# nikkolasg/ark-blst

Measured on AMD Instinct MI355X. Metric: G1 MSM points/sec, higher is better.
Workload: dtype u32; 1 GPU; G1 MSM, 2^20 random bases+scalars per GPU, bases resident, scalars in HBM; points_per_gpu=1048576, total_points=1048576, window_bits=16, num_windows=16, parallelism=base-set sharded x1, scalar_dist=uniform, precomputed_tables=False, bases_validated=True, field_repr=14 x 28-bit limbs in u32 (v_mad_u64_u32)

## Files before the change

ark-blst_amd/binding.py:

```python
from __future__ import annotations

import ctypes as C
import os
import sys

_HERE = os.path.dirname(os.path.abspath(__file__))
SCALAR_CANONICAL, SCALAR_MONTGOMERY = 0, 1
FR_MUL, FR_ADD, FR_SUB = 0, 1, 2
G1_AFF, G1_JAC, G2_AFF, G2_JAC = 96, 144, 192, 288
FP12 = 576
MAX_WINDOWS = 37


ABORT_FN = C.CFUNCTYPE(C.c_int, C.c_void_p)


class WindowInfo(C.Structure):
    _fields_ = [("window_bits", C.c_uint32), ("num_windows", C.c_uint32)]


class MsmError(RuntimeError):
    def __init__(self, code: int, where: str, detail: str = ""):
        self.code = code
        super().__init__(f"{where}: error {code} ({detail})")


class Profile(C.Structure):
    _fields_ = [(n, C.c_double) for n in ("h2d_ms", "ingest_ms", "digits_ms", "scan_ms", "scatter_ms", "accumulate_ms",
                                          "reduce_ms", "combine_ms", "d2h_ms", "host_fold_ms", "total_ms")] + [
        ("window_bits", C.c_uint32), ("num_windows", C.c_uint32), ("n", C.c_uint64), ("accumulate_adds", C.c_uint64),
        ("work_items", C.c_uint32), ("max_items_per_bucket", C.c_uint32),
        ("window_groups", C.c_uint32), ("reserved", C.c_uint32),
        ("accumulate_clock_ghz", C.c_double), ("accumulate_clock_ticks", C.c_uint64), ("accumulate_ref_ticks", C.c_uint64)]


def profile_dict(p: Profile) -> dict:
    return {f: getattr(p, f) for f, _ in Profile._fields_}


class PairingProfile(C.Structure):
    _fields_ = [(n, C.c_double) for n in ("h2d_ms", "lines_ms", "accumulate_ms", "miller_ms", "tree_ms", "host_ms", "total_ms")] + [
        ("n", C.c_uint64), ("pairs_per_accumulator", C.c_uint32), ("reserved", C.c_uint32)]


def lib_path(test_hooks: bool = False) -> str:
    return os.path.join(_HERE, "lib", "libarkblst_amd_test.so" if test_hooks else "libarkblst_amd.so")


_LIBS = {}


def load_library(test_hooks: bool = False):
    if test_hooks not in _LIBS:
        path = lib_path(test_hooks)
        if not os.path.exists(path):
            raise ImportError(f"{path} is missing: run `python -c 'import __graft_entry__ as g; g.build()'` "
                              "(hipcc --offload-arch=gfx950). There is no CPU fallback.")
        L = C.CDLL(path)
        vp, sz, u, i = C.c_void_p, C.c_size_t, C.c_uint, C.c_int
        L.mi_msm_init.argtypes = [C.POINTER(vp), C.POINTER(i), i]
        L.mi_msm_destroy.argtypes = [vp]
        L.mi_msm_destroy.restype = None
        L.mi_msm_num_devices.argtypes = [vp]
        for g in ("g1", "g2"):
            getattr(L, f"mi_msm_{g}_set_bases").argtypes = [vp, vp, sz]
            getattr(L, f"mi_msm_{g}_set_bases_precomputed").argtypes = [vp, vp, sz, u]
            getattr(L, f"mi_msm_{g}_set_bases_device").argtypes = [vp, vp, sz]
            getattr(L, f"mi_msm_{g}_set_bases_from_jacobian").argtypes = [vp, vp, sz]
            getattr(L, f"mi_msm_{g}_set_bases_from_compressed").argtypes = [vp, vp, sz, i, i, C.POINTER(sz)]
            getattr(L, f"mi_{g}_normalize_batch_device").argtypes = [vp, vp, sz, vp]
            getattr(L, f"mi_{g}_deserialize_batch_device").argtypes = [vp, vp, sz, i, i, vp, vp]
            getattr(L, f"mi_{g}_check_batch_device").argtypes = [vp, vp, sz, vp]
            getattr(L, f"mi_msm_{g}_validate_bases").argtypes = [vp, C.POINTER(sz)]
            getattr(L, f"mi_msm_{g}").argtypes = [vp, vp, vp, sz, u, vp]
            getattr(L, f"mi_msm_{g}_device").argtypes = [vp, vp, sz, u, vp]
            getattr(L, f"mi_{g}_sum").argtypes = [vp, sz, vp]
            if hasattr(L, f"mi_msm_{g}_device_windows"):
                getattr(L, f"mi_msm_{g}_device_windows").argtypes = [vp, vp, sz, u, vp, C.POINTER(WindowInfo)]
                getattr(L, f"mi_{g}_fold_windows").argtypes = [vp, sz, sz, C.POINTER(WindowInfo), vp]
            getattr(L, f"mi_msm_{g}_batch").argtypes = [vp, C.POINTER(C.c_char_p), sz, sz, u, vp]
            getattr(L, f"mi_msm_{g}_batch_device").argtypes = [vp, C.POINTER(vp), sz, sz, u, vp]
            getattr(L, f"mi_{g}_normalize_batch").argtypes = [vp, vp, sz, vp]
            if hasattr(L, f"mi_{g}_batch_mul"):
                getattr(L, f"mi_{g}_batch_mul").argtypes = [vp, vp, vp, sz, u, vp]
                getattr(L, f"mi_{g}_batch_mul_device").argtypes = [vp, vp, vp, sz, u, vp]
        if hasattr(L, "mi_batch_mul_set_window_bits"):
            L.mi_batch_mul_set_window_bits.argtypes = [vp, u]
        if hasattr(L, "mi_fr_ntt"):
            L.mi_fr_ntt.argtypes = [vp, vp, u, sz, i, vp, u, vp]
            L.mi_fr_ntt_device.argtypes = [vp, vp, u, sz, i, vp, u, vp]
            L.mi_fr_vec_op_device.argtypes = [vp, i, vp, vp, sz, u, vp]
        for g in ("g1", "g2"):
            getattr(L, f"mi_{g}_deserialize_batch").argtypes = [vp, vp, sz, i, i, vp, vp]
            getattr(L, f"mi_{g}_serialize_batch").argtypes = [vp, vp, sz, i, vp]
            getattr(L, f"mi_{g}_check_batch").argtypes = [vp, vp, sz, vp]
        L.mi_multi_miller_loop.argtypes = [vp, vp, vp, sz, vp]
        L.mi_multi_pairing.argtypes = [vp, vp, vp, sz, vp]
        L.mi_final_exponentiation.argtypes = [vp, vp]
        L.mi_msm_set_window_bits.argtypes = [vp, u]
        L.mi_msm_get_window_bits.argtypes = [vp, C.POINTER(u)]
        L.mi_msm_set_abort_check.argtypes = [vp, ABORT_FN, vp]
        L.mi_msm_set_pipeline.argtypes = [vp, C.POINTER(u), u]
        L.mi_msm_set_base_cache.argtypes = [vp, u]
        L.mi_msm_invalidate_base_cache.argtypes = [vp]
        L.mi_msm_base_cache_stats.argtypes = [vp, C.POINTER(C.c_uint64), C.POINTER(C.c_uint64), C.POINTER(u)]
        L.mi_msm_device_id.argtypes = [vp, i]
        L.mi_msm_set_profile_level.argtypes = [vp, i]
        L.mi_msm_last_profile.argtypes = [vp, C.POINTER(Profile)]
        if hasattr(L, "mi_pairing_last_profile"):
            L.mi_pairing_last_profile.argtypes = [vp, C.POINTER(PairingProfile)]
        L.mi_msm_last_error.argtypes = [vp]
        L.mi_msm_last_error.restype = C.c_char_p
        L.mi_msm_strerror.argtypes = [i]
        L.mi_msm_strerror.restype = C.c_char_p
        if test_hooks:
            L.mi_test_fp_op.argtypes = [vp, i, vp, vp, vp, sz]
            L.mi_test_field_op.argtypes = [vp, i, vp, sz, vp]
            L.mi_test_field_op_info.argtypes = [i, C.POINTER(i), C.POINTER(i), C.POINTER(i)]
            L.mi_test_field_op_info.restype = C.c_char_p
            L.mi_test_set_pairing.argtypes = [vp, u, u, i]
            L.mi_test_set_max_part.argtypes = [vp, sz]
            L.mi_test_fail_allocs.argtypes = [i]
            L.mi_test_fail_allocs.restype = None
            L.mi_test_set_no_peer.argtypes = [vp, i]
            L.mi_test_plan.argtypes = [sz, u, i, i, sz, C.POINTER(C.c_uint32)]
        _LIBS[test_hooks] = L
    return _LIBS[test_hooks]


def _buf(b):
    if b is None:
        return None, None
    if isinstance(b, int):
        return C.c_void_p(b), None
    if isinstance(b, bytes):
        return C.cast(C.c_char_p(b), C.c_void_p), b
    mv = memoryview(b)
    arr = (C.c_char * mv.nbytes).from_buffer(mv) if not mv.readonly else (C.c_char * mv.nbytes).from_buffer_copy(mv)
    return C.cast(arr, C.c_void_p), arr


def check_runtime_order():
    torch = sys.modules.get("torch")
    if torch is None or os.environ.get("ARKBLST_AMD_SKIP_RUNTIME_ORDER_CHECK"):
        return
    tlib = os.path.join(os.path.dirname(getattr(torch, "__file__", "") or ""), "lib")
    if not os.path.exists(os.path.join(tlib, "libamdhip64.so")) and not any(f.startswith("libamdhip64.so") for f in (os.listdir(tlib) if os.path.isdir(tlib) else [])):
        return
    try:
        mapped = {line.split()[-1] for line in open("/proc/self/maps") if "libamdhip64.so" in line}
    except OSError:
        return
    foreign = sorted(m for m in mapped if not os.path.realpath(m).startswith(os.path.realpath(tlib)))
    if foreign:
        raise ImportError("libarkblst_amd.so was loaded before torch: the process holds TWO HIP runtimes (" + ", ".join(sorted(mapped)) + "); torch's bundled "
                          "one under " + tlib + " then finds no devices ('No HIP GPUs are available').  Import torch BEFORE the first ark_blst_amd "
                          "context is created (INTEGRATION.md §6); ARKBLST_AMD_SKIP_RUNTIME_ORDER_CHECK=1 silences this check.")


class Context:

    def __init__(self, device_ids=None, test_hooks: bool = False):
        self._L = load_library(test_hooks)
        check_runtime_order()
        self._h = C.c_void_p()
        if device_ids is None:
            device_ids = [0]
        ids = (C.c_int * len(device_ids))(*device_ids)
        rc = self._L.mi_msm_init(C.byref(self._h), ids, len(device_ids))
        if rc != 0:
            raise MsmError(rc, "mi_msm_init", self._L.mi_msm_strerror(rc).decode())

    def close(self):
        if self._h:
            self._L.mi_msm_destroy(self._h)
            self._h = C.c_void_p()

    def __del__(self):
        try:
            self.close()
        except Exception:
            pass

    def __enter__(self):
        return self

    def __exit__(self, *a):
        self.close()

    def _check(self, rc, where):
        if rc != 0:
            raise MsmError(rc, where, (self._L.mi_msm_last_error(self._h) or b"").decode())

    def num_devices(self) -> int:
        return self._L.mi_msm_num_devices(self._h)

    def set_window_bits(self, c: int):
        self._check(self._L.mi_msm_set_window_bits(self._h, c), "mi_msm_set_window_bits")

    def set_abort_check(self, fn=None):
        self._abort_cb = ABORT_FN(lambda _user: 1 if fn() else 0) if fn else C.cast(None, ABORT_FN)
        self._check(self._L.mi_msm_set_abort_check(self._h, self._abort_cb, None), "mi_msm_set_abort_check")

    def get_window_bits(self) -> int:
        v = C.c_uint(0)
        self._check(self._L.mi_msm_get_window_bits(self._h, C.byref(v)), "mi_msm_get_window_bits")
        return v.value

    def set_pipeline(self, weights=None):
        w = list(weights or [])
        arr = (C.c_uint * max(1, len(w)))(*w)
        self._check(self._L.mi_msm_set_pipeline(self._h, arr, len(w)), "mi_msm_set_pipeline")

    def set_base_cache(self, entries: int):
        self._check(self._L.mi_msm_set_base_cache(self._h, entries), "mi_msm_set_base_cache")

    def invalidate_base_cache(self):
        self._check(self._L.mi_msm_invalidate_base_cache(self._h), "mi_msm_invalidate_base_cache")

    def base_cache_stats(self) -> dict:
        h, m, e = C.c_uint64(0), C.c_uint64(0), C.c_uint(0)
        self._check(self._L.mi_msm_base_cache_stats(self._h, C.byref(h), C.byref(m), C.byref(e)), "mi_msm_base_cache_stats")
        return {"hits": h.value, "misses": m.value, "entries": e.value}

    def device_id(self, slot: int = 0) -> int:
        return self._L.mi_msm_device_id(self._h, slot)

    def set_profile_level(self, level: int):
        self._check(self._L.mi_msm_set_profile_level(self._h, level), "mi_msm_set_profile_level")

    def set_bases(self, group: str, bases, n: int):
        p, keep = _buf(bases)
        self._check(getattr(self._L, f"mi_msm_{group}_set_bases")(self._h, p, n), f"mi_msm_{group}_set_bases")

    def set_bases_precomputed(self, group: str, bases, n: int, window_bits: int = 0):
        p, keep = _buf(bases)
        self._check(getattr(self._L, f"mi_msm_{group}_set_bases_precomputed")(self._h, p, n, window_bits),
                    f"mi_msm_{group}_set_bases_precomputed")

    def set_bases_device(self, group: str, d_bases_ptr: int, n: int):
        self._check(getattr(self._L, f"mi_msm_{group}_set_bases_device")(self._h, C.c_void_p(d_bases_ptr), n), f"mi_msm_{group}_set_bases_device")

    def set_bases_from_jacobian(self, group: str, jac, n: int):
        p, keep = _buf(jac)
        self._check(getattr(self._L, f"mi_msm_{group}_set_bases_from_jacobian")(self._h, p, n), f"mi_msm_{group}_set_bases_from_jacobian")

    def set_bases_from_compressed(self, group: str, data, n: int, compressed: bool = True, validate: bool = True) -> int:
        p, keep = _buf(data)
        rej = C.c_size_t(0)
        rc = getattr(self._L, f"mi_msm_{group}_set_bases_from_compressed")(self._h, p, n, 1 if compressed else 0, 1 if validate else 0, C.byref(rej))
        if rc != 0 and not (rc == -1 and rej.value):
            self._check(rc, f"mi_msm_{group}_set_bases_from_compressed")
        return rej.value

    def normalize_batch_device(self, group: str, d_in_ptr: int, n: int, d_out_ptr: int):
        self._check(getattr(self._L, f"mi_{group}_normalize_batch_device")(self._h, C.c_void_p(d_in_ptr), n, C.c_void_p(d_out_ptr)), f"mi_{group}_normalize_batch_device")

    def deserialize_batch_device(self, group: str, d_bytes_ptr: int, n: int, compressed: bool, validate: bool, d_out_ptr: int, d_status_ptr: int):
        self._check(getattr(self._L, f"mi_{group}_deserialize_batch_device")(self._h, C.c_void_p(d_bytes_ptr), n, 1 if compressed else 0,
                                                                              1 if validate else 0, C.c_void_p(d_out_ptr), C.c_void_p(d_status_ptr)),
                    f"mi_{group}_deserialize_batch_device")

    def check_batch_device(self, group: str, d_points_ptr: int, n: int, d_status_ptr: int):
        self._check(getattr(self._L, f"mi_{group}_check_batch_device")(self._h, C.c_void_p(d_points_ptr), n, C.c_void_p(d_status_ptr)), f"mi_{group}_check_batch_device")

    def validate_bases(self, group: str) -> int:
        bad = C.c_size_t(0)
        self._check(getattr(self._L, f"mi_msm_{group}_validate_bases")(self._h, C.byref(bad)), "mi_msm_validate_bases")
        return bad.value

    def msm(self, group: str, bases, scalars, n: int, scalar_fmt: int = SCALAR_CANONICAL) -> bytes:
        out = C.create_string_buffer(G1_JAC if group == "g1" else G2_JAC)
        pb, kb = _buf(bases)
        ps, ks = _buf(scalars)
        self._check(getattr(self._L, f"mi_msm_{group}")(self._h, pb, ps, n, scalar_fmt, out), f"mi_msm_{group}")
        return out.raw

    def msm_batch(self, group: str, scalar_vectors, n: int, scalar_fmt: int = SCALAR_CANONICAL):
        k = len(scalar_vectors)
        size = G1_JAC if group == "g1" else G2_JAC
        out = C.create_string_buffer(size * max(k, 1))
        arr = (C.c_char_p * max(k, 1))(*[bytes(v) for v in scalar_vectors])
        self._check(getattr(self._L, f"mi_msm_{group}_batch")(self._h, arr, k, n, scalar_fmt, out), f"mi_msm_{group}_batch")
        return [out.raw[size * j:size * (j + 1)] for j in range(k)]

    def msm_batch_device(self, group: str, d_scalar_ptrs, n: int, scalar_fmt: int = SCALAR_CANONICAL):
        k = len(d_scalar_ptrs)
        size = G1_JAC if group == "g1" else G2_JAC
        out = C.create_string_buffer(size * max(k, 1))
        arr = (C.c_void_p * max(k, 1))(*[C.c_void_p(p) for p in d_scalar_ptrs])
        self._check(getattr(self._L, f"mi_msm_{group}_batch_device")(self._h, arr, k, n, scalar_fmt, out), f"mi_msm_{group}_batch_device")
        return [out.raw[size * j:size * (j + 1)] for j in range(k)]

    def msm_device(self, group: str, d_scalars_ptr: int, n: int, scalar_fmt: int = SCALAR_CANONICAL) -> bytes:
        out = C.create_string_buffer(G1_JAC if group == "g1" else G2_JAC)
        self._check(getattr(self._L, f"mi_msm_{group}_device")(self._h, C.c_void_p(d_scalars_ptr), n, scalar_fmt, out),
                    f"mi_msm_{group}_device")
        return out.raw

    def msm_device_windows(self, group: str, d_scalars_ptr: int, n: int, scalar_fmt: int, d_out_ptr: int):
        info = WindowInfo()
        self._check(getattr(self._L, f"mi_msm_{group}_device_windows")(self._h, C.c_void_p(d_scalars_ptr), n, scalar_fmt,
                                                                        C.c_void_p(d_out_ptr), C.byref(info)), f"mi_msm_{group}_device_windows")
        return int(info.window_bits), int(info.num_windows)

    def normalize_batch(self, group: str, jac: bytes, into=None):
        jb, ab = (G1_JAC, G1_AFF) if group == "g1" else (G2_JAC, G2_AFF)
        n = len(jac) // jb
        if into is not None:
            po, ko = _buf(into)
            self._check(getattr(self._L, f"mi_{group}_normalize_batch")(self._h, jac, n, po), f"mi_{group}_normalize_batch")
            return into
        out = C.create_string_buffer(ab * n)
        self._check(getattr(self._L, f"mi_{group}_normalize_batch")(self._h, jac, n, out), f"mi_{group}_normalize_batch")
        return out.raw

    def batch_mul(self, group: str, base, scalars, scalar_fmt: int = SCALAR_CANONICAL, into=None):
        ab = G1_AFF if group == "g1" else G2_AFF
        n = len(scalars) // 32
        pb, kb = _buf(base)
        ps, ks = _buf(scalars)
        if into is not None:
            po, ko = _buf(into)
            self._check(getattr(self._L, f"mi_{group}_batch_mul")(self._h, pb, ps, n, scalar_fmt, po), f"mi_{group}_batch_mul")
            return into
        out = C.create_string_buffer(ab * max(n, 1))
        self._check(getattr(self._L, f"mi_{group}_batch_mul")(self._h, pb, ps, n, scalar_fmt, out), f"mi_{group}_batch_mul")
        return out.raw[:ab * n]

    def batch_mul_device(self, group: str, base, d_scalars_ptr: int, n: int, scalar_fmt: int, d_out_ptr: int):
        pb, kb = _buf(base)
        self._check(getattr(self._L, f"mi_{group}_batch_mul_device")(self._h, pb, C.c_void_p(d_scalars_ptr), n, scalar_fmt, C.c_void_p(d_out_ptr)),
                    f"mi_{group}_batch_mul_device")

    def set_batch_mul_window_bits(self, w: int):
        self._check(self._L.mi_batch_mul_set_window_bits(self._h, w), "mi_batch_mul_set_window_bits")

    def fr_ntt(self, data, log_n: int, batch: int = 1, inverse: bool = False, coset_offset=None, scalar_fmt: int = SCALAR_MONTGOMERY, into=None):
        nbytes = (batch << log_n) * 32 if 0 <= log_n <= 26 and batch > 0 else 0
        pd, kd = _buf(data)
        pc, kc = _buf(coset_offset)
        if into is not None:
            po, ko = _buf(into)
            self._check(self._L.mi_fr_ntt(self._h, pd, log_n, batch, int(inverse), pc, scalar_fmt, po), "mi_fr_ntt")
            return into
        out = C.create_string_buffer(max(nbytes, 1))
        self._check(self._L.mi_fr_ntt(self._h, pd, log_n, batch, int(inverse), pc, scalar_fmt, out), "mi_fr_ntt")
        return out.raw[:nbytes]

    def fr_ntt_device(self, d_in_ptr: int, log_n: int, batch: int, inverse: bool, coset_offset, scalar_fmt: int, d_out_ptr: int):
        pc, kc = _buf(coset_offset)
        self._check(self._L.mi_fr_ntt_device(self._h, C.c_void_p(d_in_ptr), log_n, batch, int(inverse), pc, scalar_fmt, C.c_void_p(d_out_ptr)), "mi_fr_ntt_device")

    def fr_vec_op_device(self, op: int, d_a_ptr: int, d_b_ptr: int, n: int, scalar_fmt: int, d_out_ptr: int):
        self._check(self._L.mi_fr_vec_op_device(self._h, op, C.c_void_p(d_a_ptr), C.c_void_p(d_b_ptr), n, scalar_fmt, C.c_void_p(d_out_ptr)), "mi_fr_vec_op_device")

    def deserialize_batch(self, group: str, data: bytes, compressed: bool = True, validate: bool = True, into=None):
        unit = 48 if group == "g1" else 96
        size = unit if compressed else 2 * unit
        n = len(data) // size
        if into is not None:
            po, ko = _buf(into[0])
            ps, ks = _buf(into[1])
            self._check(getattr(self._L, f"mi_{group}_deserialize_batch")(self._h, data, n, int(compressed), int(validate), po, ps),
                        f"mi_{group}_deserialize_batch")
            return into
        out = C.create_string_buffer(2 * unit * n)
        st = C.create_string_buffer(n)
        self._check(getattr(self._L, f"mi_{group}_deserialize_batch")(self._h, data, n, int(compressed), int(validate), out, st),
                    f"mi_{group}_deserialize_batch")
        return out.raw, st.raw

    def check_batch(self, group: str, points: bytes) -> bytes:
        aff = G1_AFF if group == "g1" else G2_AFF
        n = len(points) // aff
        st = C.create_string_buffer(n)
        p, keep = _buf(points)
        self._check(getattr(self._L, f"mi_{group}_check_batch")(self._h, p, n, st), f"mi_{group}_check_batch")
        return st.raw

    def serialize_batch(self, group: str, points: bytes, compressed: bool = True) -> bytes:
        unit = 48 if group == "g1" else 96
        n = len(points) // (2 * unit)
        out = C.create_string_buffer((unit if compressed else 2 * unit) * n)
        self._check(getattr(self._L, f"mi_{group}_serialize_batch")(self._h, points, n, int(compressed), out), f"mi_{group}_serialize_batch")
        return out.raw

    def g1_deserialize_batch(self, data: bytes, compressed: bool = True, validate: bool = True):
        return self.deserialize_batch("g1", data, compressed, validate)

    def g1_serialize_batch(self, points: bytes, compressed: bool = True) -> bytes:
        return self.serialize_batch("g1", points, compressed)

    def multi_miller_loop(self, g1_affine: bytes, g2_affine: bytes) -> bytes:
        n = len(g1_affine) // G1_AFF
        assert len(g1_affine) == n * G1_AFF and len(g2_affine) == n * G2_AFF, "one G2 point per G1 point"
        out = C.create_string_buffer(FP12)
        self._check(self._L.mi_multi_miller_loop(self._h, g1_affine, g2_affine, n, out), "mi_multi_miller_loop")
        return out.raw

    def multi_pairing(self, g1_affine: bytes, g2_affine: bytes) -> bytes:
        n = len(g1_affine) // G1_AFF
        assert len(g1_affine) == n * G1_AFF and len(g2_affine) == n * G2_AFF, "one G2 point per G1 point"
        out = C.create_string_buffer(FP12)
        self._check(self._L.mi_multi_pairing(self._h, g1_affine, g2_affine, n, out), "mi_multi_pairing")
        return out.raw

    def profile(self) -> dict:
        return profile_dict(self.profile_raw())

    def profile_raw(self) -> Profile:
        p = Profile()
        self._check(self._L.mi_msm_last_profile(self._h, C.byref(p)), "mi_msm_last_profile")
        return p

    def pairing_profile(self) -> dict:
        p = PairingProfile()
        self._check(self._L.mi_pairing_last_profile(self._h, C.byref(p)), "mi_pairing_last_profile")
        return {f: getattr(p, f) for f, _ in PairingProfile._fields_ if f != "reserved"}

    def test_fp_op(self, op: int, a: bytes, b: bytes) -> bytes:
        n = len(a) // 48
        out = C.create_string_buffer(48 * n)
        self._check(self._L.mi_test_fp_op(self._h, op, a, b, out, n), "mi_test_fp_op")
        return out.raw

    def test_field_op(self, op: int, data: bytes, n: int) -> bytes:
        in_slots, out_slots = C.c_int(0), C.c_int(0)
        if not self._L.mi_test_field_op_info(op, C.byref(in_slots), C.byref(out_slots), None):
            raise ValueError(f"no field op {op}")
        if len(data) != 64 * in_slots.value * n:
            raise ValueError(f"field op {op}: {n} elements take {64 * in_slots.value * n} bytes of operands, got {len(data)}")
        out = C.create_string_buffer(64 * out_slots.value * n)
        self._check(self._L.mi_test_field_op(self._h, op, data, n, out), "mi_test_field_op")
        return out.raw

    def test_field_ops(self):
        ops, a, b, k = [], C.c_int(0), C.c_int(0), C.c_int(0)
        while True:
            name = self._L.mi_test_field_op_info(len(ops), C.byref(a), C.byref(b), C.byref(k))
            if not name:
                return ops
            ops.append((name.decode(), a.value, b.value, k.value))

    def test_set_pairing(self, share: int = 0, batch: int = 0, single_lane: bool = False):
        self._check(self._L.mi_test_set_pairing(self._h, share, batch, int(single_lane)), "mi_test_set_pairing")

    def test_set_max_part(self, points: int):
        self._check(self._L.mi_test_set_max_part(self._h, points), "mi_test_set_max_part")

    def test_fail_allocs(self, count: int):
        self._L.mi_test_fail_allocs(count)

    def test_set_no_peer(self, no_peer: bool):
        self._check(self._L.mi_test_set_no_peer(self._h, int(no_peer)), "mi_test_set_no_peer")


def test_plan(n: int, forced_c: int = 0, group: str = "g1", shared: bool = False, stride: int = 0, fold: bool = False) -> dict:
    out = (C.c_uint32 * 13)()
    rc = load_library(True).mi_test_plan(n, forced_c, 0 if group == "g1" else 1, int(shared) | (2 if fold else 0), stride, out)
    if rc != 0:
        raise MsmError(rc, "mi_test_plan")
    keys = ("c", "nwin", "bwin", "coop_L", "chunk_buckets", "logT", "lo_bits", "serial", "chunks_per_win")
    d = {k: int(out[i]) for i, k in enumerate(keys)}
    d["nbuckets"] = (int(out[9]) << 32) | int(out[10])
    d["nchunks"] = int(out[11])
    d["serial_L"] = int(out[12])
    d["serial_reduce"] = d["serial"]
    return d


def final_exponentiation(f: bytes) -> bytes:
    assert len(f) == FP12
    out = C.create_string_buffer(FP12)
    rc = load_library().mi_final_exponentiation(f, out)
    if rc != 0:
        raise MsmError(rc, "mi_final_exponentiation")
    return out.raw


def _sum(group: str, partials) -> bytes:
    L = load_library()
    size = G1_JAC if group == "g1" else G2_JAC
    blob = b"".join(partials)
    assert len(blob) % size == 0
    out = C.create_string_buffer(size)
    rc = getattr(L, f"mi_{group}_sum")(blob, len(blob) // size, out)
    if rc != 0:
        raise MsmError(rc, f"mi_{group}_sum")
    return out.raw


def fold_windows(group: str, windows, n_ranks: int, rank_stride: int, window_bits: int, num_windows: int) -> bytes:
    size = G1_JAC if group == "g1" else G2_JAC
    p, keep = _buf(windows)
    assert memoryview(windows).nbytes >= n_ranks * rank_stride * size or n_ranks * num_windows == 0
    info = WindowInfo(window_bits, num_windows)
    out = C.create_string_buffer(size)
    rc = getattr(load_library(), f"mi_{group}_fold_windows")(p, n_ranks, rank_stride, C.byref(info), out)
    if rc != 0:
        raise MsmError(rc, f"mi_{group}_fold_windows")
    return out.raw


def g1_sum(partials) -> bytes:
    return _sum("g1", partials)


def g2_sum(partials) -> bytes:
    return _sum("g2", partials)


class RcclTiming(C.Structure):
    _fields_ = [("msm_ms", C.c_double), ("exchange_ms", C.c_double), ("window_bits", C.c_uint32), ("num_windows", C.c_uint32),
                ("repeats", C.c_uint32), ("bytes_per_rank", C.c_uint32)]


RCCL_UNIQUE_ID_BYTES = 128
_RCCL = []


def rccl_lib_path() -> str:
    return os.path.join(_HERE, "lib", "libarkblst_amd_rccl.so")


def load_rccl_library():
    if not _RCCL:
        load_library(False)
        path = rccl_lib_path()
        if not os.path.exists(path):
            raise ImportError(f"{path} is missing: run `python -c 'import __graft_entry__ as g; g.build()'`")
        L = C.CDLL(path)
        vp, sz, u, i = C.c_void_p, C.c_size_t, C.c_uint, C.c_int
        L.mi_rccl_get_unique_id.argtypes = [vp]
        L.mi_rccl_comm_create.argtypes = [C.POINTER(vp), vp, vp, i, i]
        L.mi_rccl_comm_attach.argtypes = [C.POINTER(vp), vp, vp]
        L.mi_rccl_comm_set_timeout_ms.argtypes = [vp, C.c_double]
        L.mi_rccl_comm_destroy.argtypes = [vp]
        L.mi_rccl_comm_destroy.restype = None
        L.mi_rccl_comm_size.argtypes = [vp]
        L.mi_rccl_comm_rank.argtypes = [vp]
        for g in ("g1", "g2"):
            getattr(L, f"mi_msm_{g}_allgather_fold").argtypes = [vp, vp, sz, u, vp]
        L.mi_rccl_last_timing.argtypes = [vp, C.POINTER(RcclTiming)]
        L.mi_rccl_last_error.restype = C.c_char_p
        _RCCL.append(L)
    return _RCCL[0]


def rccl_unique_id() -> bytes:
    L = load_rccl_library()
    buf = C.create_string_buffer(RCCL_UNIQUE_ID_BYTES)
    rc = L.mi_rccl_get_unique_id(buf)
    if rc != 0:
        raise MsmError(rc, "mi_rccl_get_unique_id", (L.mi_rccl_last_error() or b"").decode())
    return buf.raw


class RcclComm:

    def __init__(self, ctx: Context, unique_id: bytes, n_ranks: int, rank: int):
        self._L = load_rccl_library()
        self._h = C.c_void_p()
        self._ctx = ctx
        rc = self._L.mi_rccl_comm_create(C.byref(self._h), ctx._h, unique_id, n_ranks, rank)
        if rc != 0:
            raise MsmError(rc, "mi_rccl_comm_create", (self._L.mi_rccl_last_error() or b"").decode())

    def close(self):
        if self._h:
            self._L.mi_rccl_comm_destroy(self._h)
            self._h = C.c_void_p()

    def __enter__(self):
        return self

    def __exit__(self, *a):
        self.close()

    def set_timeout_ms(self, ms: float):
        rc = self._L.mi_rccl_comm_set_timeout_ms(self._h, float(ms))
        if rc != 0:
            raise MsmError(rc, "mi_rccl_comm_set_timeout_ms", (self._L.mi_rccl_last_error() or b"").decode())

    def size(self) -> int:
        return self._L.mi_rccl_comm_size(self._h)

    def rank(self) -> int:
        return self._L.mi_rccl_comm_rank(self._h)

    def allgather_fold(self, group: str, d_scalars_ptr: int, n: int, scalar_fmt: int = SCALAR_CANONICAL) -> bytes:
        out = C.create_string_buffer(G1_JAC if group == "g1" else G2_JAC)
        rc = getattr(self._L, f"mi_msm_{group}_allgather_fold")(self._h, C.c_void_p(d_scalars_ptr), n, scalar_fmt, out)
        if rc != 0:
            raise MsmError(rc, f"mi_msm_{group}_allgather_fold", (self._L.mi_rccl_last_error() or b"").decode())
        return out.raw

    def timing_raw(self) -> RcclTiming:
        t = RcclTiming()
        self._L.mi_rccl_last_timing(self._h, C.byref(t))
        return t

    def timing(self) -> dict:
        t = self.timing_raw()
        return {f: getattr(t, f) for f, _ in RcclTiming._fields_}
```

ark-blst_amd/csrc/api.hip:

```cpp
#include <random>
#include "internal.hpp"
#if defined(MI_TEST_HOOKS)
#include "test_hooks.h"
namespace mi { std::atomic<int> g_fail_allocs{0}; }
#endif

using namespace mi;

namespace {
bool cpu_ok() {
#if defined(__x86_64__)
    static const bool ok = __builtin_cpu_supports("bmi2") && __builtin_cpu_supports("adx");
    return ok;
#else
    return true;
#endif
}

template <class J, class Raw>
int fold_windows(const Raw* windows, size_t n_ranks, size_t rank_stride, const mi_window_info* info, Raw* out) {
    if (!out || !info || (n_ranks && info->num_windows && !windows)) return MI_E_INVALID;
    if (info->num_windows > MI_MAX_WINDOWS || rank_stride < info->num_windows ||
        (info->num_windows && (info->window_bits < 1 || info->window_bits > 32)))
        return MI_E_INVALID;
    if (!cpu_ok()) return MI_E_UNSUPPORTED;
    static_assert(sizeof(J) == sizeof(Raw), "host Jacobian type must be the reference's layout");
    J r = J::inf();
    for (int w = (int)info->num_windows - 1; w >= 0; w--) {
        r = r.dbl_n(info->window_bits);
        for (size_t k = 0; k < n_ranks; k++) {
            J p;
            memcpy(&p, &windows[k * rank_stride + (size_t)w], sizeof p);
            r = r.add(p);
        }
    }
    memcpy(out, &r, sizeof r);
    return MI_OK;
}
}

extern "C" {

int mi_msm_init(mi_ctx** out, const int* device_ids, int n_devices) {
    if (!out || n_devices < 0) return MI_E_INVALID;
    *out = nullptr;
    if (!cpu_ok()) return MI_E_UNSUPPORTED;
    int count = 0;
    if (hipGetDeviceCount(&count) != hipSuccess || count <= 0) return MI_E_NO_DEVICE;
    if (n_devices == 0) n_devices = device_ids ? 0 : count;
    if (n_devices <= 0 || (!device_ids && n_devices > count) || n_devices > 64) return MI_E_NO_DEVICE;
    mi_ctx* ctx = new (std::nothrow) mi_ctx();
    if (!ctx) return MI_E_NOMEM;
    int rc = guarded(ctx, [&]() -> int {
        ctx->devs.resize(n_devices);
        ctx->devs_b.resize(n_devices);
        ctx->residents.resize(n_devices);
        for (int k = 0; k < n_devices; k++) {
            int id = device_ids ? device_ids[k] : k;
            if (id < 0 || id >= count) return MI_E_NO_DEVICE;
            HIP_TRY(hipSetDevice(id));
            for (DevState* d : {&ctx->devs[k], &ctx->devs_b[k]}) {
                d->dev = id;
                d->res = ctx->residents[k].data();
                int cus = 0;
                if (hipDeviceGetAttribute(&cus, hipDeviceAttributeMultiprocessorCount, id) == hipSuccess && cus > 0) d->simds = 4u * (uint32_t)cus;
                HIP_TRY(hipStreamCreateWithFlags(&d->stream, hipStreamNonBlocking));
                HIP_TRY(hipStreamCreateWithFlags(&d->copy_stream, hipStreamNonBlocking));
                for (auto& e : d->ev) HIP_TRY(hipEventCreate(&e));
                for (auto& e : d->cev) HIP_TRY(hipEventCreate(&e));
                for (Scratch& sc : d->sc)
                    for (auto& e : sc.ev) HIP_TRY(hipEventCreate(&e));
                for (auto& row : d->iev)
                    for (auto& e : row) HIP_TRY(hipEventCreate(&e));
            }
        }
        if (const char* e = getenv("ARKBLST_AMD_TRACE")) ctx->trace = atoi(e) != 0;
        if (const char* e = getenv("ARKBLST_AMD_PIPELINE_ACC2")) ctx->pipe_two_acc_streams = atoi(e) != 0;
        if (const char* e = getenv("ARKBLST_AMD_PIPELINE")) {
            std::vector<unsigned> w;
            if (!strcmp(e, "0") || !strcmp(e, "off") || !strcmp(e, "1")) w = {1};
            else if (strcmp(e, "auto"))
                for (const char* q = e; *q;) {
                    char* end = nullptr;
                    unsigned long v = strtoul(q, &end, 10);
                    if (end == q) break;
                    w.push_back((unsigned)std::min<unsigned long>(std::max<unsigned long>(v, 1), 1000));
                    q = *end == ',' ? end + 1 : end;
                    if (*end && *end != ',') break;
                }
            if (w.size() > (size_t)MAX_GROUPS) w.resize(MAX_GROUPS);
            ctx->pipe_weights = w;
        }
        {
            std::random_device rd;
            ctx->hash_seed = ((uint64_t)rd() << 32) | rd();
            ctx->hash_mult = (((uint64_t)rd() << 32) | rd()) | 0x8000000000000001ull;
        }
        if (const char* e = getenv("ARKBLST_AMD_BASE_CACHE")) {
            long v = strtol(e, nullptr, 10);
            ctx->cache_entries = (unsigned)std::min<long>(std::max<long>(v, 0), MI_BASE_CACHE_MAX);
            ctx->cache_env = true;
        }
        if (n_devices > 1) {
            for (int l = 0; l < NLANES; l++) ctx->workers[l].reset(new DeviceWorkers((size_t)n_devices));
            for (int a = 0; a < n_devices; a++)
                for (int b = 0; b < n_devices; b++) {
                    int da = ctx->devs[a].dev, db = ctx->devs[b].dev, can = 0;
                    if (da == db) continue;
                    if (hipDeviceCanAccessPeer(&can, da, db) == hipSuccess && can) {
                        (void)hipSetDevice(da);
                        if (hipDeviceEnablePeerAccess(db, 0) != hipSuccess) (void)hipGetLastError();
                    } else {
                        (void)hipGetLastError();
                    }
                }
        }
        return MI_OK;
    });
    if (rc != MI_OK) {
        mi_msm_destroy(ctx);
        return rc;
    }
    *out = ctx;
    return MI_OK;
}

void mi_msm_destroy(mi_ctx* ctx) {
    if (!ctx) return;
    ctx->batch_workers.reset();
    for (int l = 0; l < NLANES; l++) ctx->workers[l].reset();
    for (std::vector<DevState>* lane : {&ctx->devs, &ctx->devs_b})
        for (auto& d : *lane) {
            (void)hipSetDevice(d.dev);
            if (d.stream) (void)hipStreamSynchronize(d.stream);
            if (d.acc2_stream) (void)hipStreamSynchronize(d.acc2_stream);
            if (d.aux_stream) (void)hipStreamSynchronize(d.aux_stream);
            d.for_each_buf([](DevBuf& b) { b.release(); });
            if (d.h_pairs) (void)hipHostFree(d.h_pairs);
            for (auto& e : d.ev)
                if (e) (void)hipEventDestroy(e);
            for (auto& e : d.cev)
                if (e) (void)hipEventDestroy(e);
            for (Scratch& sc : d.sc) {
                if (sc.h_meta) (void)hipHostFree(sc.h_meta);
                for (auto& e : sc.ev)
                    if (e) (void)hipEventDestroy(e);
            }
            for (auto& row : d.iev)
                for (auto& e : row)
                    if (e) (void)hipEventDestroy(e);
            if (d.d2h_stream) { (void)hipStreamSynchronize(d.d2h_stream); (void)hipStreamDestroy(d.d2h_stream); }
            if (d.aux_stream) (void)hipStreamDestroy(d.aux_stream);
            if (d.acc2_stream) (void)hipStreamDestroy(d.acc2_stream);
            if (d.copy_stream) (void)hipStreamDestroy(d.copy_stream);
            if (d.stream) (void)hipStreamDestroy(d.stream);
        }
    for (auto& v : ctx->cache) v.clear();
    if (!ctx->devs.empty()) {
        (void)hipSetDevice(ctx->devs[0].dev);
        for (FixedTable& t : ctx->fb) t.buf.release();
        for (FrTable& t : ctx->ntt_tables) { t.lo.release(); t.hi.release(); }
        ctx->ntt_scratch.release();
    }
    for (size_t k = 0; k < ctx->residents.size() && k < ctx->devs.size(); k++) {
        (void)hipSetDevice(ctx->devs[k].dev);
        for (Resident& x : ctx->residents[k]) { x.buf.release(); x.flags.release(); }
    }
    delete ctx;
}

int mi_msm_num_devices(const mi_ctx* ctx) { return ctx ? (int)ctx->devs.size() : 0; }
int mi_msm_device_id(const mi_ctx* ctx, int slot) { return ctx && slot >= 0 && (size_t)slot < ctx->devs.size() ? ctx->devs[(size_t)slot].dev : -1; }

int mi_msm_g1_set_bases(mi_ctx* ctx, const mi_g1_affine* bases, size_t n) { return g1_set_bases(ctx, bases, n, 0); }
int mi_msm_g2_set_bases(mi_ctx* ctx, const mi_g2_affine* bases, size_t n) { return g2_set_bases(ctx, bases, n, 0); }
int mi_msm_g1_set_bases_precomputed(mi_ctx* ctx, const mi_g1_affine* bases, size_t n, unsigned window_bits) {
    return g1_set_bases(ctx, bases, n, window_bits ? window_bits : 1);
}
int mi_msm_g2_set_bases_precomputed(mi_ctx* ctx, const mi_g2_affine* bases, size_t n, unsigned window_bits) {
    return g2_set_bases(ctx, bases, n, window_bits ? window_bits : 1);
}

int mi_msm_g1_validate_bases(mi_ctx* ctx, size_t* n_invalid) { return g1_validate_bases(ctx, n_invalid); }
int mi_msm_g2_validate_bases(mi_ctx* ctx, size_t* n_invalid) { return g2_validate_bases(ctx, n_invalid); }

int mi_msm_g1(mi_ctx* ctx, const mi_g1_affine* bases, const uint8_t* scalars, size_t n, unsigned scalar_fmt, mi_g1* out) {
    return g1_msm(ctx, bases, scalars, false, n, scalar_fmt, out);
}
int mi_msm_g2(mi_ctx* ctx, const mi_g2_affine* bases, const uint8_t* scalars, size_t n, unsigned scalar_fmt, mi_g2* out) {
    return g2_msm(ctx, bases, scalars, false, n, scalar_fmt, out);
}
int mi_msm_g1_device(mi_ctx* ctx, const void* d_scalars, size_t n, unsigned scalar_fmt, mi_g1* out) {
    return g1_msm(ctx, nullptr, static_cast<const uint8_t*>(d_scalars), true, n, scalar_fmt, out);
}
int mi_msm_g2_device(mi_ctx* ctx, const void* d_scalars, size_t n, unsigned scalar_fmt, mi_g2* out) {
    return g2_msm(ctx, nullptr, static_cast<const uint8_t*>(d_scalars), true, n, scalar_fmt, out);
}

int mi_msm_g1_device_windows(mi_ctx* ctx, const void* d_scalars, size_t n, unsigned scalar_fmt, void* d_out_windows, mi_window_info* info) {
    return g1_msm_windows(ctx, static_cast<const uint8_t*>(d_scalars), n, scalar_fmt, d_out_windows, info);
}
int mi_msm_g2_device_windows(mi_ctx* ctx, const void* d_scalars, size_t n, unsigned scalar_fmt, void* d_out_windows, mi_window_info* info) {
    return g2_msm_windows(ctx, static_cast<const uint8_t*>(d_scalars), n, scalar_fmt, d_out_windows, info);
}
int mi_g1_fold_windows(const mi_g1* windows, size_t n_ranks, size_t rank_stride, const mi_window_info* info, mi_g1* out) {
    return fold_windows<hostec::G1>(windows, n_ranks, rank_stride, info, out);
}
int mi_g2_fold_windows(const mi_g2* windows, size_t n_ranks, size_t rank_stride, const mi_window_info* info, mi_g2* out) {
    return fold_windows<hostec::G2>(windows, n_ranks, rank_stride, info, out);
}

int mi_msm_g1_batch(mi_ctx* ctx, const uint8_t* const* scalars, size_t k, size_t n, unsigned scalar_fmt, mi_g1* out) {
    return g1_msm_batch(ctx, scalars, false, k, n, scalar_fmt, out);
}
int mi_msm_g2_batch(mi_ctx* ctx, const uint8_t* const* scalars, size_t k, size_t n, unsigned scalar_fmt, mi_g2* out) {
    return g2_msm_batch(ctx, scalars, false, k, n, scalar_fmt, out);
}
int mi_msm_g1_batch_device(mi_ctx* ctx, const void* const* d_scalars, size_t k, size_t n, unsigned scalar_fmt, mi_g1* out) {
    return g1_msm_batch(ctx, reinterpret_cast<const uint8_t* const*>(d_scalars), true, k, n, scalar_fmt, out);
}
int mi_msm_g2_batch_device(mi_ctx* ctx, const void* const* d_scalars, size_t k, size_t n, unsigned scalar_fmt, mi_g2* out) {
    return g2_msm_batch(ctx, reinterpret_cast<const uint8_t* const*>(d_scalars), true, k, n, scalar_fmt, out);
}

int mi_g1_normalize_batch(mi_ctx* ctx, const mi_g1* in, size_t n, mi_g1_affine* out) { return g1_normalize(ctx, in, false, n, out); }
int mi_g2_normalize_batch(mi_ctx* ctx, const mi_g2* in, size_t n, mi_g2_affine* out) { return g2_normalize(ctx, in, false, n, out); }
int mi_g1_normalize_batch_device(mi_ctx* ctx, const void* d_in, size_t n, void* d_out) {
    return g1_normalize(ctx, static_cast<const mi_g1*>(d_in), true, n, static_cast<mi_g1_affine*>(d_out));
}
int mi_g2_normalize_batch_device(mi_ctx* ctx, const void* d_in, size_t n, void* d_out) {
    return g2_normalize(ctx, static_cast<const mi_g2*>(d_in), true, n, static_cast<mi_g2_affine*>(d_out));
}
int mi_msm_g1_set_bases_device(mi_ctx* ctx, const void* d_bases, size_t n) { return g1_set_bases_device(ctx, d_bases, n); }
int mi_msm_g2_set_bases_device(mi_ctx* ctx, const void* d_bases, size_t n) { return g2_set_bases_device(ctx, d_bases, n); }
int mi_msm_g1_set_bases_from_jacobian(mi_ctx* ctx, const mi_g1* points, size_t n) { return g1_set_bases_from_jacobian(ctx, points, n); }
int mi_msm_g2_set_bases_from_jacobian(mi_ctx* ctx, const mi_g2* points, size_t n) { return g2_set_bases_from_jacobian(ctx, points, n); }
int mi_msm_g1_set_bases_from_compressed(mi_ctx* ctx, const uint8_t* bytes, size_t n, int compressed, int validate, size_t* n_rejected) {
    return g1_set_bases_from_compressed(ctx, bytes, n, compressed, validate, n_rejected);
}
int mi_msm_g2_set_bases_from_compressed(mi_ctx* ctx, const uint8_t* bytes, size_t n, int compressed, int validate, size_t* n_rejected) {
    return g2_set_bases_from_compressed(ctx, bytes, n, compressed, validate, n_rejected);
}

int mi_g1_deserialize_batch(mi_ctx* ctx, const uint8_t* bytes, size_t n, int compressed, int validate, mi_g1_affine* out,
                            uint8_t* status) {
    return g1_deserialize(ctx, bytes, false, n, compressed, validate, out, status);
}
int mi_g1_deserialize_batch_device(mi_ctx* ctx, const void* d_bytes, size_t n, int compressed, int validate, void* d_out, void* d_status) {
    return g1_deserialize(ctx, static_cast<const uint8_t*>(d_bytes), true, n, compressed, validate, static_cast<mi_g1_affine*>(d_out), static_cast<uint8_t*>(d_status));
}
int mi_g2_deserialize_batch_device(mi_ctx* ctx, const void* d_bytes, size_t n, int compressed, int validate, void* d_out, void* d_status) {
    return g2_deserialize(ctx, static_cast<const uint8_t*>(d_bytes), true, n, compressed, validate, static_cast<mi_g2_affine*>(d_out), static_cast<uint8_t*>(d_status));
}
int mi_g1_serialize_batch(mi_ctx* ctx, const mi_g1_affine* points, size_t n, int compressed, uint8_t* bytes) {
    return g1_serialize(ctx, points, n, compressed, bytes);
}
int mi_g2_deserialize_batch(mi_ctx* ctx, const uint8_t* bytes, size_t n, int compressed, int validate, mi_g2_affine* out,
                            uint8_t* status) {
    return g2_deserialize(ctx, bytes, false, n, compressed, validate, out, status);
}
int mi_g2_serialize_batch(mi_ctx* ctx, const mi_g2_affine* points, size_t n, int compressed, uint8_t* bytes) {
    return g2_serialize(ctx, points, n, compressed, bytes);
}

int mi_g1_check_batch(mi_ctx* ctx, const mi_g1_affine* points, size_t n, uint8_t* status) { return g1_check_batch(ctx, points, false, n, status); }
int mi_g2_check_batch(mi_ctx* ctx, const mi_g2_affine* points, size_t n, uint8_t* status) { return g2_check_batch(ctx, points, false, n, status); }
int mi_g1_check_batch_device(mi_ctx* ctx, const void* d_points, size_t n, void* d_status) {
    return g1_check_batch(ctx, static_cast<const mi_g1_affine*>(d_points), true, n, static_cast<uint8_t*>(d_status));
}
int mi_g2_check_batch_device(mi_ctx* ctx, const void* d_points, size_t n, void* d_status) {
    return g2_check_batch(ctx, static_cast<const mi_g2_affine*>(d_points), true, n, static_cast<uint8_t*>(d_status));
}

int mi_g1_batch_mul(mi_ctx* ctx, const mi_g1_affine* base, const uint8_t* scalars, size_t n, unsigned scalar_fmt, mi_g1_affine* out) {
    return g1_batch_mul(ctx, base, scalars, false, n, scalar_fmt, out);
}
int mi_g2_batch_mul(mi_ctx* ctx, const mi_g2_affine* base, const uint8_t* scalars, size_t n, unsigned scalar_fmt, mi_g2_affine* out) {
    return g2_batch_mul(ctx, base, scalars, false, n, scalar_fmt, out);
}
int mi_g1_batch_mul_device(mi_ctx* ctx, const mi_g1_affine* base, const void* d_scalars, size_t n, unsigned scalar_fmt, void* d_out) {
    return g1_batch_mul(ctx, base, static_cast<const uint8_t*>(d_scalars), true, n, scalar_fmt, static_cast<mi_g1_affine*>(d_out));
}
int mi_g2_batch_mul_device(mi_ctx* ctx, const mi_g2_affine* base, const void* d_scalars, size_t n, unsigned scalar_fmt, void* d_out) {
    return g2_batch_mul(ctx, base, static_cast<const uint8_t*>(d_scalars), true, n, scalar_fmt, static_cast<mi_g2_affine*>(d_out));
}
int mi_batch_mul_set_window_bits(mi_ctx* ctx, unsigned window_bits) { return batch_mul_set_window_bits(ctx, window_bits); }

int mi_fr_ntt(mi_ctx* ctx, const uint8_t* in, unsigned log_n, size_t batch, int inverse, const uint8_t* coset_offset, unsigned scalar_fmt, uint8_t* out) {
    return fr_ntt(ctx, in, false, log_n, batch, inverse, coset_offset, scalar_fmt, out);
}
int mi_fr_ntt_device(mi_ctx* ctx, const void* d_in, unsigned log_n, size_t batch, int inverse, const uint8_t* coset_offset, unsigned scalar_fmt, void* d_out) {
    return fr_ntt(ctx, static_cast<const uint8_t*>(d_in), true, log_n, batch, inverse, coset_offset, scalar_fmt, static_cast<uint8_t*>(d_out));
}
int mi_fr_vec_op_device(mi_ctx* ctx, int op, const void* d_a, const void* d_b, size_t n, unsigned scalar_fmt, void* d_out) {
    return fr_vec_op(ctx, op, d_a, d_b, n, scalar_fmt, d_out);
}

int mi_multi_miller_loop(mi_ctx* ctx, const mi_g1_affine* p, const mi_g2_affine* q, size_t n, mi_fp12* out) {
    return miller(ctx, p, q, n, out, false);
}
int mi_multi_pairing(mi_ctx* ctx, const mi_g1_affine* p, const mi_g2_affine* q, size_t n, mi_fp12* out) {
    return miller(ctx, p, q, n, out, true);
}
int mi_final_exponentiation(const mi_fp12* f, mi_fp12* out) { return cpu_ok() ? final_exponentiation(f, out) : MI_E_UNSUPPORTED; }

int mi_g1_sum(const mi_g1* partials, size_t n, mi_g1* out) {
    if (!out || (n && !partials)) return MI_E_INVALID;
    if (!cpu_ok()) return MI_E_UNSUPPORTED;
    hostec::G1 r = hostec::G1::inf();
    for (size_t i = 0; i < n; i++) {
        hostec::G1 p;
        memcpy(&p, &partials[i], sizeof p);
        r = r.add(p);
    }
    memcpy(out, &r, sizeof r);
    return MI_OK;
}

int mi_g2_sum(const mi_g2* partials, size_t n, mi_g2* out) {
    if (!out || (n && !partials)) return MI_E_INVALID;
    if (!cpu_ok()) return MI_E_UNSUPPORTED;
    hostec::G2 r = hostec::G2::inf();
    for (size_t i = 0; i < n; i++) {
        hostec::G2 p;
        memcpy(&p, &partials[i], sizeof p);
        r = r.add(p);
    }
    memcpy(out, &r, sizeof r);
    return MI_OK;
}

int mi_msm_set_base_cache(mi_ctx* ctx, unsigned entries) {
    if (!ctx || entries > MI_BASE_CACHE_MAX) return fail(ctx, MI_E_INVALID, "entries must be 0..MI_BASE_CACHE_MAX");
    DeviceRestore restore;
    std::vector<std::shared_ptr<BaseCacheEntry>> dropped;
    {
        std::lock_guard<std::mutex> lk(ctx->cache_mu);
        if (ctx->cache_env) return MI_OK;
        ctx->cache_entries = entries;
        for (auto& v : ctx->cache)
            while (v.size() > entries) { dropped.push_back(v.back()); v.pop_back(); }
    }
    return MI_OK;
}

int mi_msm_invalidate_base_cache(mi_ctx* ctx) {
    if (!ctx) return MI_E_INVALID;
    DeviceRestore restore;
    std::vector<std::shared_ptr<BaseCacheEntry>> dropped;
    {
        std::lock_guard<std::mutex> lk(ctx->cache_mu);
        for (auto& v : ctx->cache) { for (auto& e : v) dropped.push_back(e); v.clear(); }
    }
    return MI_OK;
}

int mi_msm_base_cache_stats(const mi_ctx* ctx, uint64_t* hits, uint64_t* misses, unsigned* entries_in_use) {
    if (!ctx) return MI_E_INVALID;
    mi_ctx* c = const_cast<mi_ctx*>(ctx);
    std::lock_guard<std::mutex> lk(c->cache_mu);
    if (hits) *hits = c->cache_hits;
    if (misses) *misses = c->cache_misses;
    if (entries_in_use) *entries_in_use = (unsigned)(c->cache[0].size() + c->cache[1].size());
    return MI_OK;
}

int mi_msm_set_window_bits(mi_ctx* ctx, unsigned window_bits) {
    if (!ctx || (window_bits != 0 && (window_bits < 7 || window_bits > 22))) return fail(ctx, MI_E_INVALID, "window_bits must be 0 or 7..22");
    LaneLock lk(ctx, true);
    ctx->forced_c = window_bits;
    return MI_OK;
}

int mi_msm_set_abort_check(mi_ctx* ctx, int (*check)(void*), void* user) {
    if (!ctx) return MI_E_INVALID;
    LaneLock lk(ctx, true);
    ctx->abort_check = check;
    ctx->abort_user = user;
    return MI_OK;
}

int mi_msm_get_window_bits(const mi_ctx* ctx, unsigned* window_bits) {
    if (!ctx || !window_bits) return MI_E_INVALID;
    LaneLock lk(const_cast<mi_ctx*>(ctx), true);
    *window_bits = ctx->forced_c;
    return MI_OK;
}

int mi_msm_set_pipeline(mi_ctx* ctx, const unsigned* weights, unsigned n_groups) {
    if (!ctx || n_groups > (unsigned)MAX_GROUPS || (n_groups > 1 && !weights)) return fail(ctx, MI_E_INVALID, "at most 4 window groups; weights must be given for more than one");
    LaneLock lk(ctx, true);
    ctx->pipe_weights.clear();
    if (n_groups == 1) ctx->pipe_weights = {1};
    for (unsigned g = 0; n_groups > 1 && g < n_groups; g++) ctx->pipe_weights.push_back(std::min(std::max(weights[g], 1u), 1000u));
    return MI_OK;
}

int mi_msm_set_profile_level(mi_ctx* ctx, int level) {
    if (!ctx || level < 0 || level > 2) return fail(ctx, MI_E_INVALID, "profile level must be 0, 1 or 2");
    LaneLock lk(ctx, true);
    ctx->profile_level = level;
    return MI_OK;
}

int mi_msm_last_profile(const mi_ctx* ctx, mi_profile* out) {
    if (!ctx || !out) return MI_E_INVALID;
    std::lock_guard<std::mutex> lk(ctx->info_mu);
    *out = ctx->prof;
    return MI_OK;
}

int mi_pairing_last_profile(const mi_ctx* ctx, mi_pairing_profile* out) {
    if (!ctx || !out) return MI_E_INVALID;
    std::lock_guard<std::mutex> lk(ctx->info_mu);
    *out = ctx->pprof;
    return MI_OK;
}

const char* mi_msm_last_error(const mi_ctx* ctx) {
    (void)ctx;
    return tls_error().c_str();
}

const char* mi_msm_strerror(int code) {
    switch (code) {
        case MI_OK: return "ok";
        case MI_E_INVALID: return "invalid argument";
        case MI_E_NO_DEVICE: return "no usable HIP device";
        case MI_E_HIP: return "HIP runtime error";
        case MI_E_NOMEM: return "out of memory";
        case MI_E_NO_BASES: return "no resident base set";
        case MI_E_UNSUPPORTED: return "not supported on this host (the library needs an x86-64 CPU with BMI2 and ADX)";
        case MI_E_COMM: return "RCCL communication error";
        case MI_E_ABORTED: return "aborted by the caller's abort check";
        default: return "unknown error";
    }
}

#if defined(MI_TEST_HOOKS)
int mi_test_fp_op(mi_ctx* ctx, int op, const mi_fp* a, const mi_fp* b, mi_fp* out, size_t n) { return test_fp_op(ctx, op, a, b, out, n); }
int mi_test_field_op(mi_ctx* ctx, int op, const uint32_t* in, size_t n, uint32_t* out) { return test_field_op(ctx, op, in, n, out); }
const char* mi_test_field_op_info(int op, int* in_slots, int* out_slots, int* kind) { return test_field_op_info(op, in_slots, out_slots, kind); }
int mi_test_set_pairing(mi_ctx* ctx, unsigned share, unsigned batch, int single_lane) {
    if (!ctx) return MI_E_INVALID;
    LaneLock lk(ctx, true);
    ctx->test_pairing_share = share;
    ctx->test_pairing_batch = batch;
    ctx->test_pairing_single_lane = single_lane != 0;
    return MI_OK;
}
int mi_test_set_max_part(mi_ctx* ctx, size_t points) {
    if (!ctx) return MI_E_INVALID;
    LaneLock lk(ctx, true);
    ctx->test_max_part = points;
    return MI_OK;
}
void mi_test_fail_allocs(int count) { g_fail_allocs.store(count); }
int mi_test_set_no_peer(mi_ctx* ctx, int no_peer) {
    if (!ctx) return MI_E_INVALID;
    LaneLock lk(ctx, true);
    ctx->test_no_peer = no_peer != 0;
    return MI_OK;
}
int mi_test_plan(size_t n, unsigned forced_c, int group, int shared, size_t stride, uint32_t* out) {
    if (!out || n == 0) return MI_E_INVALID;
    Plan p = make_plan(n, forced_c, group == 0 ? g1_cost() : g2_cost(), (shared & 1) != 0, stride, (shared & 2) != 0);
    out[0] = p.c; out[1] = p.nwin; out[2] = p.bwin; out[3] = p.coop_L; out[4] = p.chunk_buckets; out[5] = p.logT; out[6] = p.lo_bits;
    out[7] = p.serial_reduce ? 1u : 0u; out[8] = p.chunks_per_win; out[9] = (uint32_t)(p.nbuckets >> 32); out[10] = (uint32_t)p.nbuckets;
    out[11] = (uint32_t)p.nchunks; out[12] = p.serial_reduce ? p.serial_L : 0u;
    return MI_OK;
}
#endif

}
```

ark-blst_amd/csrc/common.hpp:

```cpp
#pragma once
#include <hip/hip_runtime.h>

#include <algorithm>
#include <array>
#include <atomic>
#include <chrono>
#include <condition_variable>
#include <cstdarg>
#include <cstdio>
#include <cstdlib>
#include <cstring>
#include <functional>
#include <memory>
#include <mutex>
#include <new>
#include <string>
#include <thread>
#include <vector>

#include "../../include/arkblst_amd.h"
#include "host_curve.hpp"

namespace mi {

struct HipFail {
    std::string msg;
    bool oom = false;
    bool invalid = false;
    bool aborted = false;
};
#define HIP_TRY(expr)                                                                                     \
    do {                                                                                                  \
        hipError_t _e = (expr);                                                                           \
        if (_e != hipSuccess) {                                                                           \
            char _b[512];                                                                                 \
            snprintf(_b, sizeof _b, "%s failed: %s (%s:%d)", #expr, hipGetErrorString(_e), __FILE__, __LINE__); \
            throw ::mi::HipFail{_b, _e == hipErrorOutOfMemory};                                           \
        }                                                                                                 \
    } while (0)

#if defined(MI_TEST_HOOKS)
extern std::atomic<int> g_fail_allocs;
#endif

inline uint32_t num_windows(unsigned c, bool fold) { return (255 + c - 1) / c + ((!fold && 255 % c == 0) ? 1u : 0u); }

struct Plan {
    uint32_t c, nwin;
    uint32_t win0;
    bool fold;
    uint32_t bwin;
    uint32_t nb, coop_L, chunks_per_win, logT, lo_bits;
    uint32_t logS;
    uint32_t cls_shift;
    uint64_t nbuckets, nchunks;
    uint32_t chunk_buckets;
    bool serial_reduce;
    uint32_t serial_L;
};

struct DevBuf {
    void* p = nullptr;
    size_t cap = 0;
    void ensure(size_t bytes) {
        if (bytes <= cap) return;
#if defined(MI_TEST_HOOKS)
        if (g_fail_allocs.load() > 0 && g_fail_allocs.fetch_sub(1) > 0) throw HipFail{"injected allocation failure (test hook): out of memory", true};
#endif
        if (p) HIP_TRY(hipFree(p));
        p = nullptr;
        cap = 0;
        HIP_TRY(hipMalloc(&p, bytes));
        cap = bytes;
    }
    void release() {
        if (p) (void)hipFree(p);
        p = nullptr;
        cap = 0;
    }
    void ensure_fit(size_t bytes) {
        if (cap > 2 * bytes && cap - bytes > ((size_t)64 << 20)) release();
        ensure(bytes);
    }
};

struct Resident {
    DevBuf buf, flags;
    size_t n = 0;
    size_t lo = 0;
    uint32_t tables = 1;
    uint32_t table_c = 0;
    bool validated = false;
};

struct FixedTable {
    DevBuf buf;
    std::vector<uint8_t> key;
    unsigned w = 0;
    bool valid = false;
    uint64_t builds = 0;
};

struct FrTable {
    bool coset = false;
    unsigned log_n = 0;
    int inverse = 0;
    uint8_t key[32] = {};
    DevBuf lo, hi;
    unsigned h = 0;
    uint64_t stamp = 0;
};
constexpr size_t FR_TABLES_KEPT = 8;

struct Fp128 {
    uint64_t a = 0, b = 0;
    bool operator==(const Fp128& o) const { return a == o.a && b == o.b; }
    bool operator!=(const Fp128& o) const { return !(*this == o); }
};

struct BaseCacheEntry {
    const void* ptr = nullptr;
    size_t n = 0;
    Fp128 fp;
    uint64_t stamp = 0;
    std::vector<Resident> shard;
    std::vector<int> devs;
    ~BaseCacheEntry() {
        for (size_t k = 0; k < shard.size(); k++) {
            if (!shard[k].buf.p && !shard[k].flags.p) continue;
            (void)hipSetDevice(devs[k]);
            shard[k].buf.release();
            shard[k].flags.release();
        }
    }
};

constexpr int MAX_GROUPS = 4;
struct Scratch {
    DevBuf hist, offsets, woff, meta, sched, sorted, partial, order, item_bucket, pairs, pairs2;
    DevBuf tilecnt, tileoff, bin_tot, bin_base, binA_base, coarse, coarseA, seg_cnt, seg_base, segcnt, segoff, merge_list, merge_list2;
    uint32_t* h_meta = nullptr;
    hipEvent_t ev[8] = {};
    template <class Fn> void for_each_buf(Fn fn) {
        for (DevBuf* b : {&hist, &offsets, &woff, &meta, &sched, &sorted, &partial, &order, &item_bucket, &pairs, &pairs2, &tilecnt, &tileoff, &bin_tot,
                          &bin_base, &binA_base, &coarse, &coarseA, &seg_cnt, &seg_base, &segcnt, &segoff, &merge_list, &merge_list2})
            fn(*b);
    }
};

struct DevState {
    int dev = 0;
    uint32_t simds = 1024;
    hipStream_t stream = nullptr;
    hipStream_t copy_stream = nullptr;
    hipStream_t acc2_stream = nullptr, aux_stream = nullptr;
    hipStream_t d2h_stream = nullptr;
    hipEvent_t ev[12] = {};
    hipEvent_t cev[10] = {};
    hipEvent_t iev[4][8] = {};
    Resident* res = nullptr;
    DevBuf raw, call_bases, call_flags, scalars;
    Scratch sc[MAX_GROUPS];
    DevBuf pr_p, pr_q, pr_lvl[2], pr_raw, pr_lines;
    DevBuf io_in, io_out, io_status, nv_vals, nv_pref, nv_inv, nv_top;
    DevBuf fb_jac;
    void* h_pairs = nullptr;
    size_t h_pairs_cap = 0;
    mi_profile prof{};
    int prof_level = 1;

    void ensure_host(size_t bytes) {
        if (bytes <= h_pairs_cap) return;
        if (h_pairs) (void)hipHostFree(h_pairs);
        h_pairs = nullptr;
        h_pairs_cap = 0;
        HIP_TRY(hipHostMalloc(&h_pairs, bytes, hipHostMallocDefault));
        h_pairs_cap = bytes;
    }
    static int high_priority() {
        int lo = 0, hi = 0;
        HIP_TRY(hipDeviceGetStreamPriorityRange(&lo, &hi));
        return hi;
    }
    void ensure_pipeline_streams() {
        if (aux_stream) return;
        HIP_TRY(hipStreamCreateWithFlags(&acc2_stream, hipStreamNonBlocking));
        HIP_TRY(hipStreamCreateWithPriority(&aux_stream, hipStreamNonBlocking, high_priority()));
    }
    void ensure_d2h_stream() {
        if (!d2h_stream) HIP_TRY(hipStreamCreateWithPriority(&d2h_stream, hipStreamNonBlocking, high_priority()));
    }
    template <class Fn> void for_each_buf(Fn fn) {
        for (DevBuf* b : {&raw, &call_bases, &call_flags, &scalars, &pr_p, &pr_q, &pr_lvl[0], &pr_lvl[1], &pr_raw, &pr_lines, &io_in, &io_out, &io_status,
                          &nv_vals, &nv_pref, &nv_inv, &nv_top, &fb_jac})
            fn(*b);
        for (Scratch& s : sc) s.for_each_buf(fn);
    }
};

constexpr int NLANES = 2;
class HashPool;

class DeviceWorkers {
public:
    explicit DeviceWorkers(size_t n) : slots_(n) {
        for (size_t k = 0; k < n; k++) threads_.emplace_back([this, k] { loop(k); });
    }
    ~DeviceWorkers() {
        {
            std::lock_guard<std::mutex> lk(mu_);
            stop_ = true;
        }
        cv_.notify_all();
        for (auto& t : threads_) t.join();
    }
    DeviceWorkers(const DeviceWorkers&) = delete;
    DeviceWorkers& operator=(const DeviceWorkers&) = delete;
    size_t size() const { return threads_.size(); }
    void run(const std::function<void(size_t)>& fn) {
        std::unique_lock<std::mutex> lk(mu_);
        fn_ = &fn;
        pending_ = slots_.size();
        for (auto& s : slots_) s = true;
        cv_.notify_all();
        done_cv_.wait(lk, [&] { return pending_ == 0; });
        fn_ = nullptr;
    }

private:
    void loop(size_t k) {
        for (;;) {
            const std::function<void(size_t)>* fn;
            {
                std::unique_lock<std::mutex> lk(mu_);
                cv_.wait(lk, [&] { return stop_ || slots_[k]; });
                if (stop_) return;
                slots_[k] = false;
                fn = fn_;
            }
            (*fn)(k);
            {
                std::lock_guard<std::mutex> lk(mu_);
                if (--pending_ == 0) done_cv_.notify_all();
            }
        }
    }
    std::vector<std::thread> threads_;
    std::vector<char> slots_;
    std::mutex mu_;
    std::condition_variable cv_, done_cv_;
    const std::function<void(size_t)>* fn_ = nullptr;
    size_t pending_ = 0;
    bool stop_ = false;
};

}

struct mi_ctx {
    std::vector<mi::DevState> devs;
    std::vector<mi::DevState> devs_b;
    std::vector<std::array<mi::Resident, 2>> residents;
    std::unique_ptr<mi::DeviceWorkers> workers[mi::NLANES];
    std::unique_ptr<mi::DeviceWorkers> batch_workers;
    std::mutex batch_mu;
    std::mutex lane_mu;
    std::condition_variable lane_cv;
    bool lane_busy[mi::NLANES] = {false, false};
    mutable std::mutex info_mu;
    unsigned forced_c = 0;
    unsigned fb_forced_w = 0;
    mi::FixedTable fb[2];
    std::vector<mi::FrTable> ntt_tables;
    uint64_t ntt_clock = 0;
    mi::DevBuf ntt_scratch;
    std::vector<unsigned> pipe_weights;
    int (*abort_check)(void*) = nullptr;
    void* abort_user = nullptr;
    bool pipe_two_acc_streams = false;
    bool trace = false;
    std::mutex cache_mu;
    unsigned cache_entries = 0;
    bool cache_env = false;
    uint64_t cache_clock = 0, cache_hits = 0, cache_misses = 0;
    std::vector<std::shared_ptr<mi::BaseCacheEntry>> cache[2];
    uint64_t hash_seed = 0, hash_mult = 0xD6E8FEB86659FD93ull;
    std::shared_ptr<mi::HashPool> hash_pool[mi::NLANES];
    int profile_level = 1;
    mi_profile prof{};
    mi_pairing_profile pprof{};
    std::string err;
#if defined(MI_TEST_HOOKS)
    unsigned test_pairing_share = 0, test_pairing_batch = 0;
    bool test_pairing_single_lane = false;
    size_t test_max_part = 0;
    bool test_no_peer = false;
#endif
};

namespace mi {

struct HashKey { uint64_t seed = 0, mult = 0xD6E8FEB86659FD93ull; };
struct SliceHash { uint64_t h[4]; };
inline SliceHash hash_slice(const uint8_t* p, size_t bytes, uint64_t slice, const HashKey& key) {
    const uint64_t K = key.mult | 1u, seed = key.seed + slice * 0x9E3779B97F4A7C15ull;
    SliceHash s{{0x9E3779B97F4A7C15ull ^ seed, 0xC2B2AE3D27D4EB4Full + seed, 0x165667B19E3779F9ull ^ (seed << 1), 0x27D4EB2F165667C5ull + (seed << 2)}};
    size_t i = 0;
    for (; i + 32 <= bytes; i += 32) {
        uint64_t w[4];
        memcpy(w, p + i, 32);
        for (int t = 0; t < 4; t++) {
            s.h[t] = (s.h[t] ^ w[t]) * K;
            s.h[t] ^= s.h[t] >> 32;
        }
    }
    if (i < bytes) {
        uint64_t w[4] = {0, 0, 0, 0};
        memcpy(w, p + i, bytes - i);
        for (int t = 0; t < 4; t++) {
            s.h[t] = (s.h[t] ^ w[t] ^ (uint64_t)(bytes - i)) * K;
            s.h[t] ^= s.h[t] >> 32;
        }
    }
    return s;
}
inline Fp128 fold_slices(const SliceHash* s, size_t count, uint64_t total_bytes) {
    Fp128 r{0x243F6A8885A308D3ull ^ total_bytes, 0x13198A2E03707344ull + total_bytes};
    for (size_t k = 0; k < count; k++)
        for (int t = 0; t < 4; t++) {
            r.a = (r.a ^ s[k].h[t]) * 0xD6E8FEB86659FD93ull;
            r.a ^= r.a >> 29;
            r.b = (r.b + s[k].h[t]) * 0x9FB21C651E98DF25ull;
            r.b ^= r.b >> 31;
        }
    return r;
}
constexpr size_t HASH_SLICE_MIN = (size_t)1 << 20;
inline size_t hash_slices(size_t bytes, size_t threads) { return std::max<size_t>(1, std::min(threads, bytes / HASH_SLICE_MIN)); }
inline Fp128 content_fingerprint(const uint8_t* p, size_t bytes, size_t threads, const HashKey& key = HashKey{}) {
    const size_t S = hash_slices(bytes, threads);
    std::vector<SliceHash> part(S);
    for (size_t k = 0; k < S; k++) {
        const size_t lo = (bytes / 32 * k / S) * 32, hi = k + 1 == S ? bytes : (bytes / 32 * (k + 1) / S) * 32;
        part[k] = hash_slice(p + lo, hi - lo, (uint64_t)k, key);
    }
    return fold_slices(part.data(), S, bytes);
}

class HashPool {
public:
    explicit HashPool(size_t threads, const HashKey& key = HashKey{}) : key_(key), part_(std::max<size_t>(1, threads)) {
        for (size_t k = 0; k < part_.size(); k++) threads_.emplace_back([this, k] { loop(k); });
    }
    ~HashPool() {
        {
            std::lock_guard<std::mutex> lk(mu_);
            stop_ = true;
        }
        cv_.notify_all();
        for (auto& t : threads_) t.join();
    }
    HashPool(const HashPool&) = delete;
    HashPool& operator=(const HashPool&) = delete;
    size_t threads() const { return part_.size(); }
    bool busy() const { return busy_; }
    void start(const uint8_t* p, size_t bytes) {
        std::lock_guard<std::mutex> lk(mu_);
        p_ = p; bytes_ = bytes;
        slices_ = hash_slices(bytes, part_.size());
        pending_ = slices_;
        gen_++;
        busy_ = true;
        cv_.notify_all();
    }
    Fp128 finish() {
        std::unique_lock<std::mutex> lk(mu_);
        done_cv_.wait(lk, [&] { return pending_ == 0; });
        busy_ = false;
        return fold_slices(part_.data(), slices_, bytes_);
    }

private:
    void loop(size_t k) {
        uint64_t seen = 0;
        for (;;) {
            const uint8_t* p;
            size_t bytes, S;
            {
                std::unique_lock<std::mutex> lk(mu_);
                cv_.wait(lk, [&] { return stop_ || gen_ != seen; });
                if (stop_) return;
                seen = gen_;
                p = p_; bytes = bytes_; S = slices_;
            }
            if (k >= S) continue;
            const size_t lo = (bytes / 32 * k / S) * 32, hi = k + 1 == S ? bytes : (bytes / 32 * (k + 1) / S) * 32;
            const SliceHash h = hash_slice(p + lo, hi - lo, (uint64_t)k, key_);
            {
                std::lock_guard<std::mutex> lk(mu_);
                part_[k] = h;
                if (--pending_ == 0) done_cv_.notify_all();
            }
        }
    }
    const HashKey key_;
    std::vector<SliceHash> part_;
    std::vector<std::thread> threads_;
    std::mutex mu_;
    std::condition_variable cv_, done_cv_;
    const uint8_t* p_ = nullptr;
    size_t bytes_ = 0, slices_ = 0, pending_ = 0;
    uint64_t gen_ = 0;
    bool stop_ = false, busy_ = false;
};
inline size_t hash_pool_threads() {
    if (const char* e = getenv("ARKBLST_AMD_HASH_THREADS")) return (size_t)std::min(16l, std::max(1l, atol(e)));
    return std::min<size_t>(6, std::max<size_t>(1, std::thread::hardware_concurrency() / 3));
}

inline bool cache_begin(mi_ctx* ctx, int idx, const void* ptr, size_t n, std::shared_ptr<BaseCacheEntry>& candidate) {
    std::lock_guard<std::mutex> lk(ctx->cache_mu);
    if (!ctx->cache_entries) return false;
    for (auto& e : ctx->cache[idx])
        if (e->ptr == ptr && e->n == n && (!candidate || e->stamp > candidate->stamp)) candidate = e;
    return true;
}
inline std::shared_ptr<BaseCacheEntry> cache_find(mi_ctx* ctx, int idx, const void* ptr, size_t n, const Fp128& fp) {
    std::lock_guard<std::mutex> lk(ctx->cache_mu);
    for (auto& e : ctx->cache[idx])
        if (e->ptr == ptr && e->n == n && e->fp == fp) return e;
    return nullptr;
}
inline void cache_finish(mi_ctx* ctx, int idx, const std::shared_ptr<BaseCacheEntry>& hit, const std::shared_ptr<BaseCacheEntry>& fill, const Fp128& fp) {
    std::vector<std::shared_ptr<BaseCacheEntry>> dropped;
    std::lock_guard<std::mutex> lk(ctx->cache_mu);
    auto& v = ctx->cache[idx];
    if (hit) {
        hit->stamp = ++ctx->cache_clock;
        ctx->cache_hits++;
        return;
    }
    ctx->cache_misses++;
    if (!fill) return;
    fill->fp = fp;
    bool dup = false;
    for (auto& e : v) dup = dup || (e->ptr == fill->ptr && e->n == fill->n && e->fp == fill->fp);
    if (dup || !ctx->cache_entries) return;
    fill->stamp = ++ctx->cache_clock;
    v.push_back(fill);
    while (v.size() > ctx->cache_entries) {
        size_t old = 0;
        for (size_t q = 1; q < v.size(); q++)
            if (v[q]->stamp < v[old]->stamp) old = q;
        dropped.push_back(v[old]);
        v.erase(v.begin() + (long)old);
    }
}

struct LaneLock {
    mi_ctx* c;
    int lane;
    LaneLock(mi_ctx* ctx, bool exclusive) : c(ctx), lane(-1) {
        std::unique_lock<std::mutex> lk(c->lane_mu);
        if (exclusive) {
            c->lane_cv.wait(lk, [&] { return !c->lane_busy[0] && !c->lane_busy[1]; });
            c->lane_busy[0] = c->lane_busy[1] = true;
        } else {
            c->lane_cv.wait(lk, [&] { return !c->lane_busy[0] || !c->lane_busy[1]; });
            lane = c->lane_busy[0] ? 1 : 0;
            c->lane_busy[lane] = true;
        }
    }
    ~LaneLock() {
        {
            std::lock_guard<std::mutex> lk(c->lane_mu);
            if (lane < 0) c->lane_busy[0] = c->lane_busy[1] = false;
            else c->lane_busy[lane] = false;
        }
        c->lane_cv.notify_all();
    }
    LaneLock(const LaneLock&) = delete;
    LaneLock& operator=(const LaneLock&) = delete;
    std::vector<DevState>& devs() { return lane == 1 ? c->devs_b : c->devs; }
    DeviceWorkers* workers() { return c->workers[lane == 1 ? 1 : 0].get(); }
};

inline bool abort_requested(const mi_ctx* ctx) { return ctx->abort_check && ctx->abort_check(ctx->abort_user) != 0; }

inline void set_prof(mi_ctx* ctx, const mi_profile& p) {
    std::lock_guard<std::mutex> lk(ctx->info_mu);
    ctx->prof = p;
}

inline double ev_ms(hipEvent_t a, hipEvent_t b) {
    float ms = 0;
    HIP_TRY(hipEventElapsedTime(&ms, a, b));
    return ms;
}

inline std::string& tls_error() {
    static thread_local std::string e;
    return e;
}

inline int fail(mi_ctx* ctx, int code, const std::string& msg) {
    tls_error() = msg;
    if (ctx) {
        std::lock_guard<std::mutex> lk(ctx->info_mu);
        ctx->err = msg;
    }
    return code;
}

struct DeviceRestore {
    int dev = -1;
    DeviceRestore() {
        if (hipGetDevice(&dev) != hipSuccess) { dev = -1; (void)hipGetLastError(); }
    }
    ~DeviceRestore() {
        if (dev >= 0) (void)hipSetDevice(dev);
    }
    DeviceRestore(const DeviceRestore&) = delete;
    DeviceRestore& operator=(const DeviceRestore&) = delete;
};

template <class Fn>
int guarded(mi_ctx* ctx, Fn fn) {
    DeviceRestore restore;
    try {
        return fn();
    } catch (const HipFail& e) {
        bool oom = e.oom || e.msg.find("out of memory") != std::string::npos;
        return fail(ctx, e.aborted ? MI_E_ABORTED : e.invalid ? MI_E_INVALID : oom ? MI_E_NOMEM : MI_E_HIP, e.msg);
    } catch (const std::bad_alloc&) {
        return fail(ctx, MI_E_NOMEM, "host allocation failed");
    } catch (const std::exception& e) {
        return fail(ctx, MI_E_HIP, std::string("unexpected exception: ") + e.what());
    } catch (...) {
        return fail(ctx, MI_E_HIP, "unexpected exception");
    }
}

struct PartErr {
    int code = MI_OK;
    std::string msg;
};
template <class Fn>
void guarded_part(PartErr& e, Fn fn) noexcept {
    try {
        fn();
    } catch (const HipFail& f) {
        e.code = f.aborted ? MI_E_ABORTED : f.invalid ? MI_E_INVALID : (f.oom || f.msg.find("out of memory") != std::string::npos) ? MI_E_NOMEM : MI_E_HIP;
        e.msg = f.msg;
    } catch (const std::bad_alloc&) {
        e.code = MI_E_NOMEM;
        e.msg = "host allocation failed";
    } catch (const std::exception& x) {
        e.code = MI_E_HIP;
        e.msg = std::string("unexpected exception: ") + x.what();
    } catch (...) {
        e.code = MI_E_HIP;
        e.msg = "unexpected exception";
    }
}

template <class Fn>
void for_each_device(LaneLock& lane, size_t g, Fn fn) {
    DeviceWorkers* w = lane.workers();
    if (g == 1 || !w) {
        for (size_t k = 0; k < g; k++) fn(k);
    } else {
        std::function<void(size_t)> f = fn;
        w->run(f);
    }
}

inline int device_of_ptr(const void* p, const char* what, size_t align = 16) {
    if (reinterpret_cast<uintptr_t>(p) & (align - 1))
        throw HipFail{std::string(what) + " must be " + std::to_string(align) + "-byte aligned", false, true};
    hipPointerAttribute_t a{};
    hipError_t e = hipPointerGetAttributes(&a, p);
    if (e != hipSuccess) (void)hipGetLastError();
    if (e != hipSuccess || a.type == hipMemoryTypeUnregistered)
        throw HipFail{std::string(what) + " is not device memory known to this HIP runtime (a host pointer, or memory allocated through a "
                      "second HIP runtime in this process: see INTEGRATION.md, load order)", false, true};
    return a.device;
}
inline void shard_range(size_t n, size_t g, size_t k, size_t& lo, size_t& hi) {
    size_t per = (n + g - 1) / g;
    lo = std::min(n, k * per);
    hi = std::min(n, lo + per);
}

}
```

ark-blst_amd/csrc/kernels_common.cuh:

```cuda
#pragma once
#include <hip/hip_runtime.h>
#include "ec.cuh"
#include "coop_fp2.cuh"
#include "fr.cuh"

namespace msmk {

using fp28::Fp;
using fp28::NL;

__device__ __forceinline__ void load_fp16(Fp& r, const uint32_t* p) {
    const uint4* q = reinterpret_cast<const uint4*>(p);
    uint4 a = q[0], b = q[1], c = q[2], d = q[3];
    r.l[0] = a.x; r.l[1] = a.y; r.l[2] = a.z; r.l[3] = a.w;
    r.l[4] = b.x; r.l[5] = b.y; r.l[6] = b.z; r.l[7] = b.w;
    r.l[8] = c.x; r.l[9] = c.y; r.l[10] = c.z; r.l[11] = c.w;
    r.l[12] = d.x; r.l[13] = d.y;
}
__device__ __forceinline__ void store_fp16(uint32_t* p, const Fp& r, uint32_t w14 = 0, uint32_t w15 = 0) {
    uint4* q = reinterpret_cast<uint4*>(p);
    q[0] = make_uint4(r.l[0], r.l[1], r.l[2], r.l[3]);
    q[1] = make_uint4(r.l[4], r.l[5], r.l[6], r.l[7]);
    q[2] = make_uint4(r.l[8], r.l[9], r.l[10], r.l[11]);
    q[3] = make_uint4(r.l[12], r.l[13], w14, w15);
}
__device__ __forceinline__ Fp shfl_down_fp(const Fp& a, int d) {
    Fp r;
#pragma unroll
    for (int k = 0; k < NL; k++) r.l[k] = __shfl_down(a.l[k], d, 64);
    return r;
}
__device__ __forceinline__ void fp_from_raw(Fp& r, const uint32_t* raw) {
    uint32_t w[12];
#pragma unroll
    for (int k = 0; k < 12; k++) w[k] = raw[k];
    r = fp28::fp_from_blst(w);
}
__device__ __forceinline__ uint32_t fp_to_raw(uint32_t* out, const Fp& a, bool keep) {
    uint32_t w[12], any = 0;
    fp28::fp_to_blst(w, a);
#pragma unroll
    for (int k = 0; k < 12; k++) { out[k] = keep ? w[k] : 0u; any |= w[k]; }
    return any;
}

__device__ __forceinline__ void fp_unpack_raw(Fp& r, const uint32_t* raw) {
    uint32_t w[12];
#pragma unroll
    for (int k = 0; k < 12; k++) w[k] = raw[k];
    r = fp28::fp_unpack384(w);
}
__device__ __forceinline__ void fp_pack_raw(uint32_t* out, const Fp& a, bool keep) {
    uint32_t w[12];
    fp28::fp_pack384(w, fp28::fp_canon_2p(a));
#pragma unroll
    for (int k = 0; k < 12; k++) out[k] = keep ? w[k] : 0u;
}

template <class E> struct ElemIO;
template <> struct ElemIO<Fp> {
    static constexpr int SLOT = 16, RAW = 12;
    static __device__ __forceinline__ void load(Fp& r, const uint32_t* p) { load_fp16(r, p); }
    static __device__ __forceinline__ void store(uint32_t* p, const Fp& r, uint32_t flag = 0) { store_fp16(p, r, 0, flag); }
    static __device__ __forceinline__ Fp shfl_down(const Fp& a, int d) { return shfl_down_fp(a, d); }
    static __device__ __forceinline__ void from_raw(Fp& r, const uint32_t* raw) { fp_from_raw(r, raw); }
    static __device__ __forceinline__ uint32_t to_raw(uint32_t* out, const Fp& a, bool keep) { return fp_to_raw(out, a, keep); }
    static __device__ __forceinline__ void unpack_raw(Fp& r, const uint32_t* raw) { fp_unpack_raw(r, raw); }
    static __device__ __forceinline__ void pack_raw(uint32_t* out, const Fp& a, bool keep) { fp_pack_raw(out, a, keep); }
};
template <> struct ElemIO<ec::Fp2> {
    static constexpr int SLOT = 32, RAW = 24;
    static __device__ __forceinline__ void load(ec::Fp2& r, const uint32_t* p) { load_fp16(r.c0, p); load_fp16(r.c1, p + 16); }
    static __device__ __forceinline__ void store(uint32_t* p, const ec::Fp2& r, uint32_t flag = 0) {
        store_fp16(p, r.c0);
        store_fp16(p + 16, r.c1, 0, flag);
    }
    static __device__ __forceinline__ ec::Fp2 shfl_down(const ec::Fp2& a, int d) {
        return ec::Fp2{shfl_down_fp(a.c0, d), shfl_down_fp(a.c1, d)};
    }
    static __device__ __forceinline__ void from_raw(ec::Fp2& r, const uint32_t* raw) { fp_from_raw(r.c0, raw); fp_from_raw(r.c1, raw + 12); }
    static __device__ __forceinline__ uint32_t to_raw(uint32_t* out, const ec::Fp2& a, bool keep) {
        return fp_to_raw(out, a.c0, keep) | fp_to_raw(out + 12, a.c1, keep);
    }
    static __device__ __forceinline__ void unpack_raw(ec::Fp2& r, const uint32_t* raw) { fp_unpack_raw(r.c0, raw); fp_unpack_raw(r.c1, raw + 12); }
    static __device__ __forceinline__ void pack_raw(uint32_t* out, const ec::Fp2& a, bool keep) { fp_pack_raw(out, a.c0, keep); fp_pack_raw(out + 12, a.c1, keep); }
};

struct G1C {
    using F = ec::FpOps;
    using FA = ec::FpOpsInline;
    using FR = ec::FpOpsInlinePS;
    static constexpr int OCC = 2;
};
struct G2C {
    using F = ec::Fp2Ops;
    using FA = ec::Fp2OpsInline;
    using FR = ec::Fp2OpsInline;
    static constexpr int OCC = 2;
};
template <class C> struct Geo {
    using E = typename C::F::E;
    static constexpr int SLOT = ElemIO<E>::SLOT;
    static constexpr int PT_WORDS = 2 * SLOT, BK_WORDS = 3 * SLOT;
    static constexpr int RAW_AFF = 2 * ElemIO<E>::RAW, RAW_JAC = 3 * ElemIO<E>::RAW;
};
constexpr int G1_PT_WORDS = Geo<G1C>::PT_WORDS, G1_BK_WORDS = Geo<G1C>::BK_WORDS;
constexpr int G2_PT_WORDS = Geo<G2C>::PT_WORDS, G2_BK_WORDS = Geo<G2C>::BK_WORDS;

__device__ __noinline__ void add_inplace(ec::Proj<ec::FpOps>& a, const ec::Proj<ec::FpOps>& b) { ec::proj_add<ec::FpOpsInline>(a, b); }
__device__ __noinline__ void add_inplace(ec::Proj<ec::Fp2Ops>& a, const ec::Proj<ec::Fp2Ops>& b) { ec::proj_add<ec::Fp2Ops>(a, b); }

template <class C_>
struct OneLane {
    using C = C_;
    using F = typename C::F;
    using FA = typename C::FA;
    using E = typename F::E;
    static constexpr int LANES = 1;
    static constexpr bool TAIL_OUT_OF_LINE = false;
    static __device__ __forceinline__ uint32_t unit(uint32_t gid) { return gid; }
    static __device__ __forceinline__ uint32_t lane() { return 0; }
    static __device__ __forceinline__ bool leader() { return true; }
    static __device__ __forceinline__ uint32_t unit_or(uint32_t v) { return v; }
    static __device__ __forceinline__ void cold_add(ec::Proj<F>& a, const ec::Proj<F>& b) { ec::proj_add<F>(a, b); }
};
static __device__ __noinline__ void coop_add_inplace(ec::Proj<CoopF2>& a, const ec::Proj<CoopF2>& b) { ec::proj_add<CoopF2>(a, b); }
struct LanePairG2 {
    using C = G2C;
    using F = CoopF2;
    using FA = CoopF2A;
    using E = Fp;
    static constexpr int LANES = 2;
    static constexpr bool TAIL_OUT_OF_LINE = true;
    static __device__ __forceinline__ uint32_t unit(uint32_t gid) { return gid >> 1; }
    static __device__ __forceinline__ uint32_t lane() { return threadIdx.x & 1u; }
    static __device__ __forceinline__ bool leader() { return lane() == 0; }
    static __device__ __forceinline__ uint32_t unit_or(uint32_t v) { return CoopF2::pair_or(v); }
    static __device__ __forceinline__ void cold_add(ec::Proj<F>& a, const ec::Proj<F>& b) { coop_add_inplace(a, b); }
};
template <class C> struct HotViewOf { using V = OneLane<C>; };
template <> struct HotViewOf<G2C> { using V = LanePairG2; };
template <class C> using HotView = typename HotViewOf<C>::V;
template <class V>
__device__ __forceinline__ void load_xy(typename V::E& x, typename V::E& y, const uint32_t* pts, uint32_t ent) {
    using IO = ElemIO<typename V::E>;
    const uint32_t* p = pts + (size_t)(ent & 0x7fffffffu) * Geo<typename V::C>::PT_WORDS + IO::SLOT * V::lane();
    IO::load(x, p);
    IO::load(y, p + IO::SLOT * V::LANES);
}
template <class V>
__device__ __forceinline__ ec::Proj<typename V::F> load_proj(const uint32_t* bucket) {
    using IO = ElemIO<typename V::E>;
    const uint32_t* p = bucket + IO::SLOT * V::lane();
    ec::Proj<typename V::F> r;
    IO::load(r.x, p); IO::load(r.y, p + IO::SLOT * V::LANES); IO::load(r.z, p + 2 * IO::SLOT * V::LANES);
    return r;
}
template <class V>
__device__ __forceinline__ void store_proj(uint32_t* bucket, const ec::Proj<typename V::F>& r) {
    using IO = ElemIO<typename V::E>;
    uint32_t* o = bucket + IO::SLOT * V::lane();
    IO::store(o, r.x); IO::store(o + IO::SLOT * V::LANES, r.y); IO::store(o + 2 * IO::SLOT * V::LANES, r.z);
}
template <class C>
__device__ __forceinline__ ec::Proj<typename C::F> load_bucket(const uint32_t* p) { return load_proj<OneLane<C>>(p); }
template <class C>
__device__ __forceinline__ void store_bucket(uint32_t* p, const ec::Proj<typename C::F>& r) { store_proj<OneLane<C>>(p, r); }
template <class V>
__device__ __forceinline__ void store_jac_raw(uint32_t* out, const ec::Proj<typename V::F>& p) {
    using F = typename V::F;
    using IO = ElemIO<typename V::E>;
    constexpr int R = IO::RAW;
    uint32_t* o = out + R * V::lane();
    uint32_t zw[R];
    const uint32_t any = V::unit_or(IO::to_raw(zw, p.z, true));
    const typename V::E zz = F::sqr(p.z);
    IO::to_raw(o, F::mul(p.x, p.z), any != 0);
    IO::to_raw(o + R * V::LANES, F::mul(p.y, zz), any != 0);
#pragma unroll
    for (int k = 0; k < R; k++) o[2 * R * V::LANES + k] = zw[k];
}

using fr::load_scalar;

#ifndef MI_AUX_PRIO
#define MI_AUX_PRIO 3
#endif
__device__ __forceinline__ void aux_priority() {
#if MI_AUX_PRIO
    __builtin_amdgcn_s_setprio(MI_AUX_PRIO);
#endif
}

constexpr uint32_t MERGE_FAN = 4;
constexpr uint32_t MERGE_META = 32;
constexpr uint32_t CLK_META = 24;

struct WaveClock {
    static __device__ __forceinline__ void start(uint32_t* own_slot) {
        if ((threadIdx.x & 63u) == 0) {
            const unsigned long long t0 = clock64(), w0 = wall_clock64();
            reinterpret_cast<unsigned long long*>(own_slot)[0] = t0;
            reinterpret_cast<unsigned long long*>(own_slot)[1] = w0;
        }
    }
    static __device__ __forceinline__ void stop(const uint32_t* own_slot, uint32_t* meta) {
        if ((threadIdx.x & 63u) == 0) {
            const unsigned long long t0 = reinterpret_cast<const unsigned long long*>(own_slot)[0], w0 = reinterpret_cast<const unsigned long long*>(own_slot)[1];
            atomicAdd(reinterpret_cast<unsigned long long*>(meta + CLK_META), clock64() - t0);
            atomicAdd(reinterpret_cast<unsigned long long*>(meta + CLK_META + 2), wall_clock64() - w0);
        }
    }
};

__device__ __forceinline__ uint32_t item_size_log(uint32_t cnt, uint32_t logT, uint32_t logS) { return cnt > (1u << logT) ? logS : logT; }

__device__ __forceinline__ uint32_t scalar_bits(const uint32_t (&s)[8], uint32_t off, uint32_t c) {
    uint32_t w = off >> 5, sh = off & 31;
    uint32_t lo = 0, hi = 0;
#pragma unroll
    for (int k = 0; k < 8; k++) {
        lo = (w == (uint32_t)k) ? s[k] : lo;
        hi = (w + 1 == (uint32_t)k) ? s[k] : hi;
    }
    uint64_t v = ((uint64_t)hi << 32) | lo;
    return (uint32_t)(v >> sh) & ((1u << c) - 1u);
}

template <class Fn>
__device__ __forceinline__ void for_each_digit(const uint32_t (&s)[8], bool flip, uint32_t c, uint32_t nwin, Fn f) {
    uint32_t carry = 0, half = 1u << (c - 1);
    for (uint32_t w = 0; w < nwin; w++) {
        uint32_t raw = scalar_bits(s, w * c, c) + carry;
        bool neg = raw > half;
        carry = neg ? 1u : 0u;
        uint32_t mag = neg ? (1u << c) - raw : raw;
        if (mag != 0) f(w, mag - 1, neg != flip);
    }
}

template <int CB, class Fn>
__device__ __forceinline__ void for_each_digit_static(const uint32_t (&s)[8], bool flip, uint32_t w0, uint32_t w1, Fn f) {
    constexpr uint32_t NW = (255 + CB - 1) / CB + (255 % CB == 0 ? 1 : 0), HALF = 1u << (CB - 1), MASKC = (1u << CB) - 1u;
    uint32_t carry = 0;
#pragma unroll
    for (uint32_t w = 0; w < NW; w++) {
        constexpr uint32_t dummy = 0; (void)dummy;
        const uint32_t off = w * CB, wi = off >> 5, sh = off & 31;
        uint32_t v = wi < 8 ? s[wi < 8 ? wi : 0] >> sh : 0u;
        if (sh + CB > 32 && wi + 1 < 8) v |= s[wi + 1 < 8 ? wi + 1 : 0] << (32 - sh);
        uint32_t raw = (v & MASKC) + carry;
        bool neg = raw > HALF;
        carry = neg ? 1u : 0u;
        uint32_t mag = neg ? (1u << CB) - raw : raw;
        if (w >= w0 && w < w1 && mag != 0) f(w, mag - 1, neg != flip);
    }
}

}
```

ark-blst_amd/csrc/msm_sort.hip:

```cpp
#include <cmath>
#include "internal.hpp"
#include "sort_kernels.cuh"

namespace mi {

namespace {
struct ReduceCost { double coop_steps = 0, coop_rounds = 0, serial_steps = 0, serial_rounds = 0; };

bool reduce_geometry(Plan& p, const CurveCost& cc, ReduceCost& rc) {
    const uint32_t c = p.c;
    const uint32_t log_ll = (uint32_t)cc.log_ll;
    if (c - 1 < log_ll) return false;
    {
        double best = 1e300;
        const uint32_t max_L = std::min<uint32_t>(64, std::max<uint32_t>(1, p.nb >> log_ll));
        uint32_t coop_L_lo = 1, coop_L_hi = max_L;
#if defined(MI_TEST_HOOKS)
        if (const char* e = getenv("MI_TEST_COOP_L")) coop_L_lo = coop_L_hi = (uint32_t)std::min<int>((int)max_L, std::max(1, atoi(e)));
#endif
        for (uint32_t L = coop_L_lo; L <= coop_L_hi; L++) {
            const uint64_t chunks = (uint64_t)((p.nb + (L << log_ll) - 1) / (L << log_ll)) * p.bwin;
            const double rounds = (double)((chunks + cc.max_chunks - 1) / cc.max_chunks);
            uint32_t bits = 0, ones = 0;
            for (uint32_t v = L; v; v >>= 1) { bits++; ones += v & 1u; }
            const double steps = 2.0 * L + 2.0 * log_ll + (bits - 1) + (ones - 1) + 1.0;
            if (rounds * steps < best) { best = rounds * steps; p.coop_L = L; rc.coop_steps = steps; rc.coop_rounds = rounds; }
        }
    }
    p.chunk_buckets = p.coop_L << log_ll;
    p.serial_reduce = cc.serial_buckets != 0 && p.nbuckets >= cc.serial_buckets && c - 1 >= 6;
    uint32_t serial_L_lo = 8, serial_L_hi = 64;
#if defined(MI_TEST_HOOKS)
    if (const char* e = getenv("MI_TEST_SERIAL_MIN_BUCKETS")) p.serial_reduce = cc.serial_buckets != 0 && p.nbuckets >= (uint64_t)atoll(e) && c - 1 >= 6;
    if (const char* e = getenv("MI_TEST_SERIAL_L")) serial_L_lo = serial_L_hi = (uint32_t)std::min(64, std::max(1, atoi(e)));
#endif
    p.chunks_per_win = (p.nb + p.chunk_buckets - 1) / p.chunk_buckets;
    p.serial_L = 0;
    if (p.serial_reduce) {
        double best = 1e300;
        for (uint32_t L = serial_L_lo; L <= serial_L_hi; L++) {
            const uint64_t lanes = (uint64_t)((p.nb + L - 1) / L) * p.bwin;
            const double rounds = std::ceil(std::ceil((double)lanes / 64.0) / (double)cc.max_chunks);
            uint32_t bits = 0, ones = 0;
            for (uint32_t v = L; v; v >>= 1) { bits++; ones += v & 1u; }
            const double steps = 2.0 * L + (bits - 1) + (ones - 1);
            if (rounds * steps < best) { best = rounds * steps; p.serial_L = L; rc.serial_steps = steps; rc.serial_rounds = rounds; }
        }
        p.chunk_buckets = p.serial_L; p.coop_L = 0;
        p.chunks_per_win = (p.nb + p.serial_L - 1) / p.serial_L;
    }
    p.nchunks = (uint64_t)p.chunks_per_win * p.bwin;
    return true;
}
}

Plan make_plan(size_t n, unsigned forced_c, const CurveCost& cc, bool shared, size_t stride, bool fold) {
    Plan best{};
    double best_cost = 1e300;
    for (unsigned c = 7; c <= 22; c++) {
        if (forced_c && c != forced_c) continue;
        Plan p{};
        p.c = c;
        p.win0 = 0;
        p.fold = fold;
        p.nwin = num_windows(c, fold);
        uint32_t idx_bits = 1;
        const uint64_t nidx = shared ? (uint64_t)std::max(stride, n) * p.nwin : n;
        while ((1ull << idx_bits) < nidx) idx_bits++;
        if (idx_bits > 30) continue;
        uint32_t lo_bits = std::min<uint32_t>(std::min<uint32_t>(8, c - 1), 31 - idx_bits);
        if (((1u << (c - 1)) >> lo_bits) > msmk::SORT_MAX_COUNTERS) continue;
        p.lo_bits = lo_bits;
        if ((uint64_t)n * p.nwin >= (1ull << 32)) continue;
        p.nb = 1u << (c - 1);
        p.bwin = shared ? 1 : p.nwin;
        p.nbuckets = (uint64_t)p.nb * p.bwin;
        ReduceCost rc;
        if (!reduce_geometry(p, cc, rc)) continue;
        const double coop_steps = rc.coop_steps, coop_rounds = rc.coop_rounds, serial_steps = rc.serial_steps, serial_rounds = rc.serial_rounds;
        const double entries = (double)n * p.nwin;
        double mean = entries / (double)p.nbuckets;
        int top_bits = std::max(0, std::min<int>((fold ? 254 : 255) - (int)c * ((int)p.nwin - 1), (int)c - 1));
        double per_bucket = (double)n / (double)(1u << top_bits) + (shared ? mean : 0.0);
        const double typical = per_bucket > mean && per_bucket <= 4.0 * mean ? per_bucket : mean;
        p.logT = 5;
        while ((double)(1u << p.logT) < 2.0 * typical && p.logT < 20) p.logT++;
        p.cls_shift = p.logT > 6 ? p.logT - 6 : 0;
        const double walk = 0.2 * ((entries + 0.2 * (double)p.nbuckets) / cc.add_per_us) / cc.lane_add_us;
        while (p.logT < 20 && (double)(2u << p.logT) <= walk) p.logT++;
        const double T = (double)(1u << p.logT);
        p.logS = std::max<uint32_t>(4, p.logT - 2);
        double merge_total_us = 0;
        if (per_bucket > T) {
            const double lanes_at_once = (double)cc.max_chunks * (double)(1u << cc.comb_log_ll);
            double per = per_bucket / (double)(1u << p.logS), all = per * (double)(1u << top_bits);
            for (; per > 1.0; per /= (double)msmk::MERGE_FAN, all /= (double)msmk::MERGE_FAN)
                merge_total_us += std::max(cc.merge_us, std::ceil(all / (double)msmk::MERGE_FAN / lanes_at_once) * (msmk::MERGE_FAN - 1) * cc.step_us);
            merge_total_us += 1.6e-4 * (double)n;
        }
        const double tail = mean + 4.5 * std::sqrt(mean);
        double item_len = std::min(T, std::max(tail, per_bucket > T ? (double)(1u << p.logS) : per_bucket + 3.0 * std::sqrt(per_bucket)));
        if (per_bucket > T && top_bits < 4) item_len = T;
        int levels = 0;
        for (uint32_t m = p.chunks_per_win; m > 1; m = (m + (1u << cc.comb_log_ll) - 1) >> cc.comb_log_ll) levels++;
        const double reduce_us = p.serial_reduce ? serial_rounds * serial_steps * cc.serial_step_us
                                                 : coop_rounds * coop_steps * (p.nchunks <= 1000 ? cc.lone_step_us : cc.step_us);
        const double comb_chain = (2.0 * cc.comb_log_ll + 1.0) * cc.comb_step_us;
        const double comb_us = std::max(1, levels) * (comb_chain + 8.0) +
                               std::max(0.0, std::ceil((double)(p.nchunks >> cc.comb_log_ll) / 2048.0) - 1.0) * comb_chain;
        const double nonempty = (double)p.nbuckets * (1.0 - std::exp(-mean));
        double acc_adds = entries - nonempty + 1.2 * (double)p.nbuckets;
        const double wave_rounds = (double)p.nbuckets / 64.0 / (double)cc.max_chunks;
        if (wave_rounds < 4.0) acc_adds *= 1.0 + 0.5 * (std::ceil(wave_rounds) - wave_rounds) / std::max(wave_rounds, 0.25);
        const double lane_us = cc.lane_add_us * ((double)p.nbuckets / cc.acc_wave_items <= 1024.0 ? cc.lone_lane : 1.0);
        const double drain_us = 0.5 * std::max(0.0, mean - 3.0 * std::sqrt(mean)) * cc.lane_add_us;
        double cost = std::max(acc_adds / cc.add_per_us + drain_us, item_len * lane_us) + merge_total_us + reduce_us + comb_us +
                      entries / 41000.0 + (double)p.nbuckets / 1e4 + (shared ? 20.0 : 100.0);
        if (cost < best_cost) {
            best_cost = cost;
            best = p;
        }
    }
    return best;
}

std::vector<Plan> split_plan(const Plan& pl, const CurveCost& cc, size_t n, bool shared, const std::vector<unsigned>& weights) {
    (void)cc;
    std::vector<unsigned> w = weights;
    if (w.empty()) {
        w = {1};
    }
    if (w.size() > (size_t)MAX_GROUPS) w.resize(MAX_GROUPS);
    if (w.size() > pl.nwin) w.resize(pl.nwin);
    if (shared || w.size() <= 1 || pl.bwin != pl.nwin) return {pl};
    const size_t G = w.size();
    uint64_t sum = 0;
    for (unsigned& x : w) { x = std::max(1u, x); sum += x; }
    std::vector<uint32_t> cnt(G);
    std::vector<double> frac(G);
    uint32_t used = 0;
    for (size_t g = 0; g < G; g++) {
        const double exact = (double)pl.nwin * w[g] / (double)sum;
        cnt[g] = std::max<uint32_t>(1, (uint32_t)exact);
        frac[g] = exact - (double)cnt[g];
        used += cnt[g];
    }
    while (used < pl.nwin) {
        size_t b = 0;
        for (size_t g = 1; g < G; g++) if (frac[g] > frac[b]) b = g;
        cnt[b]++; frac[b] -= 1.0; used++;
    }
    while (used > pl.nwin) {
        size_t b = 0;
        for (size_t g = 1; g < G; g++) if (cnt[g] > cnt[b]) b = g;
        cnt[b]--; used--;
    }
    std::vector<Plan> out;
    uint32_t top = pl.nwin;
    for (size_t g = 0; g < G; g++) {
        Plan p = pl;
        p.nwin = p.bwin = cnt[g];
        top -= cnt[g];
        p.win0 = top;
        p.nbuckets = (uint64_t)p.nb * p.bwin;
        p.nchunks = (uint64_t)p.chunks_per_win * p.bwin;
        out.push_back(p);
    }
    return out;
}

namespace {

template <int LO, int HI, class F>
void dispatch_c(uint32_t c, const char* out_of_range, F&& f) {
    if constexpr (LO > HI) {
        throw HipFail{out_of_range};
    } else {
        if (c == LO) f(std::integral_constant<int, LO>{});
        else dispatch_c<LO + 1, HI>(c, out_of_range, f);
    }
}
template <bool SCATTER>
void launch_coarse(uint32_t c, dim3 grid, dim3 block, hipStream_t s, const uint32_t* scalars, const uint8_t* flags, const msmk::SortGeom& g,
                   uint32_t* tilecnt, const uint32_t* tileoff, const uint32_t* bin_base, uint32_t* coarse) {
    dispatch_c<7, 22>(c, "window_bits out of range", [&](auto cb) {
        hipLaunchKernelGGL((msmk::k_coarse<SCATTER, decltype(cb)::value>), grid, block, 0, s, scalars, flags, g, tilecnt, tileoff, bin_base, coarse);
    });
}
template <bool SCATTER>
void launch_coarseA(uint32_t c, dim3 grid, dim3 block, hipStream_t s, const uint32_t* scalars, const uint8_t* flags, const msmk::SortGeom& g,
                    uint32_t* tilecnt, const uint32_t* tileoff, const uint32_t* binA_base, uint2* coarseA) {
    dispatch_c<17, 22>(c, "three-level sort: window_bits out of range", [&](auto cb) {
        hipLaunchKernelGGL((msmk::k_coarseA<SCATTER, decltype(cb)::value>), grid, block, 0, s, scalars, flags, g, tilecnt, tileoff, binA_base, coarseA);
    });
}
void launch_coarse_staged(uint32_t c, bool co, dim3 grid, hipStream_t s, const uint32_t* scalars, const uint8_t* flags, const msmk::SortGeom& g,
                          const uint32_t* tilecnt, const uint32_t* tileoff, const uint32_t* bin_base, uint32_t* coarse) {
    dispatch_c<7, 16>(c, "staged coarse scatter: window_bits out of range", [&](auto cb) {
        constexpr int CB = decltype(cb)::value;
        if (co) hipLaunchKernelGGL((msmk::k_coarse_staged_co<CB>), grid, dim3(256), msmk::COARSE_STAGED_CO_LDS, s, scalars, flags, g, tilecnt, tileoff, bin_base, coarse);
        else hipLaunchKernelGGL((msmk::k_coarse_staged<CB>), grid, dim3(512), 0, s, scalars, flags, g, tilecnt, tileoff, bin_base, coarse);
    });
}

}

void sort_and_schedule(DevState& d, Scratch& sc, hipStream_t s, const Plan& pl, const uint32_t* d_scalars, const uint8_t* d_flags, size_t n, unsigned fmt,
                       bool shared_buckets, size_t stride, SortOut& out, const uint8_t* host_scalars, bool under_accumulate) {
    const dim3 digit_block_big(under_accumulate ? 256 : 1024);
    const size_t entries_cap = (size_t)n * pl.nwin;
    sc.hist.ensure(pl.nbuckets * 4);
    sc.offsets.ensure((pl.nbuckets + 1) * 4);
    sc.woff.ensure((pl.nbuckets + 1) * 4);
    sc.meta.ensure(msmk::MERGE_META * 4);
    sc.sorted.ensure(entries_cap * 4);
    if (!sc.h_meta) HIP_TRY(hipHostMalloc((void**)&sc.h_meta, 32, hipHostMallocDefault));

    const bool phases = d.prof_level >= 2;
    if (phases) HIP_TRY(hipEventRecord(sc.ev[0], s));
    auto feed_and_count = [&](msmk::SortGeom& gg, auto&& count_tiles) {
        const uint32_t K = host_scalars ? std::min<uint32_t>(8, std::max<uint32_t>(1, std::min<uint32_t>(gg.tiles, (uint32_t)(n >> 16)))) : 1;
        if (host_scalars) HIP_TRY(hipEventRecord(d.cev[0], d.copy_stream));
        for (uint32_t j = 0; j < K; j++) {
            const uint32_t t0 = (uint32_t)((uint64_t)gg.tiles * j / K), t1 = (uint32_t)((uint64_t)gg.tiles * (j + 1) / K);
            if (host_scalars) {
                const size_t p0 = (size_t)t0 * gg.tile_pts, p1 = std::min<size_t>(n, (size_t)t1 * gg.tile_pts);
                HIP_TRY(hipMemcpyAsync((char*)const_cast<uint32_t*>(d_scalars) + p0 * 32, host_scalars + p0 * 32, (p1 - p0) * 32, hipMemcpyHostToDevice,
                                       d.copy_stream));
                HIP_TRY(hipEventRecord(d.cev[1 + j], d.copy_stream));
                HIP_TRY(hipStreamWaitEvent(s, d.cev[1 + j], 0));
            }
            gg.tile0 = t0;
            if (t1 > t0) count_tiles(t1 - t0);
        }
        gg.tile0 = 0;
        if (host_scalars) {
            HIP_TRY(hipEventRecord(d.cev[9], d.copy_stream));
            HIP_TRY(hipStreamWaitEvent(s, d.cev[9], 0));
        }
    };
    msmk::SortGeom g{};
    g.n = (uint32_t)n; g.fmt = fmt | (pl.fold ? 2u : 0u); g.c = pl.c; g.nwin = pl.nwin; g.win0 = pl.win0;
    g.shared = shared_buckets ? 1u : 0u;
    g.stride = (uint32_t)stride;
    g.lo_bits = pl.lo_bits;
    g.H = pl.nb >> g.lo_bits;
    g.nbins = pl.bwin * g.H;
    sc.bin_base.ensure((size_t)(g.nbins + 1) * 4);
    sc.coarse.ensure(entries_cap * 4);
    const uint32_t segs_cap = g.nbins + (uint32_t)(entries_cap / msmk::FINE_SEG) + 1;
    const bool three_level = !shared_buckets && pl.c >= 17;
    {
        size_t seg_words = (size_t)segs_cap * (1u << g.lo_bits), bins = g.nbins;
        if (three_level) {
            const uint32_t nbinsA = pl.nwin * msmk::A_BINS;
            const size_t segs_capA = nbinsA + entries_cap / msmk::FINE_SEG + 1;
            seg_words = std::max(seg_words, segs_capA << ((pl.c - 1 - msmk::A_BITS) - pl.lo_bits));
            bins = std::max<size_t>(bins, nbinsA);
        }
        sc.seg_cnt.ensure(bins * 4);
        sc.seg_base.ensure((bins + 1) * 4);
        sc.segcnt.ensure(seg_words * 4);
        sc.segoff.ensure(seg_words * 4);
    }
    if (three_level) {
        const uint32_t nbinsA = pl.nwin * msmk::A_BINS;
        const uint32_t mid_bits = (pl.c - 1 - msmk::A_BITS) - pl.lo_bits, M = 1u << mid_bits;
        if (nbinsA > 512 || M > msmk::MID_MAX || nbinsA * M != g.nbins) throw HipFail{"three-level sort: geometry"};
        g.wgroup = pl.nwin; g.ngroups = 1;
        g.tile_pts = (uint32_t)std::min<size_t>(8192, (n + 1023) / 1024 * 1024);
        g.tiles = (uint32_t)((n + g.tile_pts - 1) / g.tile_pts);
        const uint32_t segs_capA = nbinsA + (uint32_t)(entries_cap / msmk::FINE_SEG) + 1;
        sc.tilecnt.ensure((size_t)g.tiles * nbinsA * 4);
        sc.tileoff.ensure((size_t)g.tiles * nbinsA * 4);
        sc.bin_tot.ensure((size_t)nbinsA * 4);
        sc.binA_base.ensure((size_t)(nbinsA + 1) * 4);
        sc.coarseA.ensure(entries_cap * 8);
        feed_and_count(g, [&](uint32_t ntiles) {
            launch_coarseA<false>(pl.c, dim3(ntiles), digit_block_big, s, d_scalars, d_flags, g, (uint32_t*)sc.tilecnt.p, (const uint32_t*)nullptr,
                                  (const uint32_t*)nullptr, (uint2*)nullptr);
        });
        hipLaunchKernelGGL(msmk::k_colscan, dim3((nbinsA + 255) / 256), dim3(256), 0, s, (const uint32_t*)sc.tilecnt.p, nbinsA, g.tiles,
                           (uint32_t*)sc.tileoff.p, (uint32_t*)sc.bin_tot.p);
        hipLaunchKernelGGL(msmk::k_binscan, dim3(1), dim3(1024), 0, s, (const uint32_t*)sc.bin_tot.p, nbinsA, (uint32_t*)sc.binA_base.p);
        launch_coarseA<true>(pl.c, dim3(g.tiles), digit_block_big, s, d_scalars, d_flags, g, (uint32_t*)sc.tilecnt.p, (const uint32_t*)sc.tileoff.p,
                             (const uint32_t*)sc.binA_base.p, (uint2*)sc.coarseA.p);
        hipLaunchKernelGGL(msmk::k_seg_count, dim3((nbinsA + 255) / 256), dim3(256), 0, s, (const uint32_t*)sc.binA_base.p, nbinsA,
                           (uint32_t*)sc.seg_cnt.p);
        hipLaunchKernelGGL(msmk::k_binscan, dim3(1), dim3(1024), 0, s, (const uint32_t*)sc.seg_cnt.p, nbinsA, (uint32_t*)sc.seg_base.p);
        hipLaunchKernelGGL(msmk::k_mid_count, dim3(segs_capA), dim3(256), 0, s, (const uint2*)sc.coarseA.p, (const uint32_t*)sc.binA_base.p,
                           (const uint32_t*)sc.seg_base.p, nbinsA, pl.lo_bits, mid_bits, (uint32_t*)sc.segcnt.p);
        hipLaunchKernelGGL(msmk::k_mid_scan, dim3(nbinsA), dim3(512), 0, s, (const uint32_t*)sc.binA_base.p, (const uint32_t*)sc.seg_base.p, mid_bits,
                           (const uint32_t*)sc.segcnt.p, (uint32_t*)sc.segoff.p, (uint32_t*)sc.bin_base.p, nbinsA);
        hipLaunchKernelGGL(msmk::k_mid_scatter, dim3(segs_capA), dim3(256), msmk::MID_SCATTER_LDS, s, (const uint2*)sc.coarseA.p, (const uint32_t*)sc.binA_base.p,
                           (const uint32_t*)sc.seg_base.p, nbinsA, pl.lo_bits, mid_bits, (const uint32_t*)sc.segcnt.p, (const uint32_t*)sc.segoff.p,
                           (uint32_t*)sc.coarse.p);
    } else {
    const bool staged = !shared_buckets && g.H <= 128 && pl.c <= 16 && n >= 4096;
    uint32_t coarse_block;
    if (staged) {
        g.wgroup = std::min<uint32_t>(std::min<uint32_t>(pl.nwin, 16), msmk::COARSE_STAGE_BINS / g.H);
        g.tile_pts = under_accumulate ? (msmk::COARSE_STAGE_CO / g.wgroup) / 256 * 256 : (msmk::COARSE_STAGE / g.wgroup) / 512 * 512;
        coarse_block = under_accumulate ? 256 : 512;
    } else {
        size_t want = std::max<size_t>(std::max<size_t>(4096, n / 512), (size_t)64 * g.H / (shared_buckets ? pl.nwin : 1));
        g.tile_pts = (uint32_t)((std::min(want, n) + 1023) / 1024 * 1024);
        coarse_block = g.tile_pts >= 16384 && !under_accumulate ? 1024 : 256;
        g.wgroup = shared_buckets ? pl.nwin : std::max<uint32_t>(1, std::min<uint32_t>(pl.nwin, msmk::SORT_MAX_COUNTERS / g.H));
    }
    g.tiles = (uint32_t)((n + g.tile_pts - 1) / g.tile_pts);
    g.ngroups = (pl.nwin + g.wgroup - 1) / g.wgroup;
    sc.tilecnt.ensure((size_t)g.tiles * g.nbins * 4);
    sc.tileoff.ensure((size_t)g.tiles * g.nbins * 4);
    sc.bin_tot.ensure((size_t)g.nbins * 4);
    feed_and_count(g, [&](uint32_t ntiles) {
        launch_coarse<false>(pl.c, dim3(ntiles, g.ngroups), dim3(coarse_block), s, d_scalars, d_flags, g, (uint32_t*)sc.tilecnt.p,
                             (const uint32_t*)nullptr, (const uint32_t*)nullptr, (uint32_t*)nullptr);
    });
    hipLaunchKernelGGL(msmk::k_colscan, dim3((g.nbins + 255) / 256), dim3(256), 0, s, (const uint32_t*)sc.tilecnt.p, g.nbins, g.tiles,
                       (uint32_t*)sc.tileoff.p, (uint32_t*)sc.bin_tot.p);
    hipLaunchKernelGGL(msmk::k_binscan, dim3(1), dim3(1024), 0, s, (const uint32_t*)sc.bin_tot.p, g.nbins, (uint32_t*)sc.bin_base.p);
    if (staged)
        launch_coarse_staged(pl.c, under_accumulate, dim3(g.tiles, g.ngroups), s, d_scalars, d_flags, g, (const uint32_t*)sc.tilecnt.p, (const uint32_t*)sc.tileoff.p,
                             (const uint32_t*)sc.bin_base.p, (uint32_t*)sc.coarse.p);
    else
        launch_coarse<true>(pl.c, dim3(g.tiles, g.ngroups), dim3(coarse_block), s, d_scalars, d_flags, g, (uint32_t*)sc.tilecnt.p,
                            (const uint32_t*)sc.tileoff.p, (const uint32_t*)sc.bin_base.p, (uint32_t*)sc.coarse.p);
    }
    if (phases) HIP_TRY(hipEventRecord(sc.ev[1], s));
    hipLaunchKernelGGL(msmk::k_seg_count, dim3((g.nbins + 255) / 256), dim3(256), 0, s, (const uint32_t*)sc.bin_base.p, g.nbins,
                       (uint32_t*)sc.seg_cnt.p);
    hipLaunchKernelGGL(msmk::k_binscan, dim3(1), dim3(1024), 0, s, (const uint32_t*)sc.seg_cnt.p, g.nbins, (uint32_t*)sc.seg_base.p);
    hipLaunchKernelGGL(msmk::k_fine_count, dim3(segs_cap), dim3(256), 0, s, (const uint32_t*)sc.coarse.p, (const uint32_t*)sc.bin_base.p,
                       (const uint32_t*)sc.seg_base.p, g, (uint32_t*)sc.segcnt.p);
    hipLaunchKernelGGL(msmk::k_fine_scan, dim3(g.nbins), dim3(256), 0, s, (const uint32_t*)sc.seg_base.p, g, (const uint32_t*)sc.segcnt.p,
                       (uint32_t*)sc.segoff.p, (uint32_t*)sc.hist.p);
    hipLaunchKernelGGL(msmk::k_fine_scatter, dim3(segs_cap), dim3(256), msmk::FINE_SCATTER_LDS, s, (const uint32_t*)sc.coarse.p, (const uint32_t*)sc.bin_base.p,
                       (const uint32_t*)sc.seg_base.p, g, (const uint32_t*)sc.segcnt.p, (const uint32_t*)sc.segoff.p, (uint32_t*)sc.sorted.p);
    if (phases) HIP_TRY(hipEventRecord(sc.ev[2], s));
    const uint32_t sched_nt = under_accumulate ? 512 : 1024;
    uint32_t per_blk = 4 * sched_nt;
    while ((pl.nbuckets + per_blk - 1) / per_blk > msmk::SCHED_MAX_BLK) per_blk <<= 1;
    uint32_t nblk = (uint32_t)((pl.nbuckets + per_blk - 1) / per_blk);
    const size_t items_cap = pl.nbuckets + (entries_cap >> pl.logS) + 1;
    out.items_cap = items_cap;
    sc.sched.ensure((size_t)(3 + msmk::SCHED_CLASSES) * nblk * 4);
    sc.order.ensure(items_cap * 4);
    sc.item_bucket.ensure(items_cap * 4);
    sc.merge_list.ensure((items_cap / 2 + 1) * 4);
    sc.merge_list2.ensure((items_cap / 2 + 1) * 4);
    uint32_t* blk_e = (uint32_t*)sc.sched.p;
    uint32_t* blk_i = blk_e + nblk;
    uint32_t* blk_max = blk_i + nblk;
    uint32_t* blk_cls = blk_max + nblk;
    const uint32_t packed = pl.logT | (pl.cls_shift << 8) | (pl.logS << 16);
    auto schedule = [&](auto nt_tag) {
        constexpr uint32_t NT = decltype(nt_tag)::value;
        hipLaunchKernelGGL(msmk::k_sched1<NT>, dim3(nblk), dim3(NT), 0, s, (const uint32_t*)sc.hist.p, (uint32_t)pl.nbuckets, per_blk, packed, nblk, blk_e, blk_i, blk_cls,
                           blk_max);
        hipLaunchKernelGGL(msmk::k_sched2<NT>, dim3(1), dim3(NT), 0, s, nblk, blk_e, blk_i, blk_cls, (const uint32_t*)blk_max, (uint32_t*)sc.meta.p);
        hipLaunchKernelGGL(msmk::k_sched3<NT>, dim3(nblk), dim3(NT), 0, s, (const uint32_t*)sc.hist.p, (uint32_t)pl.nbuckets, per_blk, packed, nblk, (const uint32_t*)blk_e,
                           (const uint32_t*)blk_i, (const uint32_t*)blk_cls, (uint32_t*)sc.offsets.p, (uint32_t*)sc.woff.p, (uint32_t*)sc.order.p,
                           (uint32_t*)sc.item_bucket.p, (uint32_t*)sc.merge_list.p, (uint32_t*)sc.meta.p);
    };
    if (under_accumulate) schedule(std::integral_constant<uint32_t, 512>{});
    else schedule(std::integral_constant<uint32_t, 1024>{});
    HIP_TRY(hipMemcpyAsync(sc.h_meta, sc.meta.p, 32, hipMemcpyDeviceToHost, s));
    HIP_TRY(hipEventRecord(sc.ev[3], s));
}

void read_schedule(Scratch& sc, SortOut& out) {
    HIP_TRY(hipEventSynchronize(sc.ev[3]));
    HIP_TRY(hipGetLastError());
    out.nitems = sc.h_meta[0];
    out.max_items = sc.h_meta[1];
    out.entries = sc.h_meta[2];
    out.nlist = sc.h_meta[3];
    out.nsplit = sc.h_meta[4];
    if ((uint64_t)out.nlist > out.items_cap / 2 + 1) throw HipFail{"schedule produced a longer merge list than its bound"};
    if (out.nitems > out.items_cap) throw HipFail{"schedule produced more work items than its bound"};
}

}
```

ark-blst_amd/csrc/sort_kernels.cuh:

```cuda
#pragma once
#include "kernels_common.cuh"

namespace msmk {

struct SortGeom {
    uint32_t n, fmt, c, nwin;
    uint32_t win0;
    uint32_t lo_bits, H;
    uint32_t tiles, tile_pts;
    uint32_t tile0;
    uint32_t wgroup, ngroups;
    uint32_t nbins;
    uint32_t shared, stride;
};
constexpr uint32_t SORT_MAX_COUNTERS = 16384;

template <uint32_t NT, uint32_t PER = 1, class... Arr>
__device__ __forceinline__ void block_scan_inclusive(Arr&... arrays) {
    const uint32_t t = threadIdx.x;
    for (uint32_t d = 1; d < NT * PER; d <<= 1) {
        uint32_t x[PER][sizeof...(arrays)];
#pragma unroll
        for (uint32_t r = 0; r < PER; r++) {
            const uint32_t k = t + NT * r;
            int i = 0;
            ((x[r][i++] = k >= d ? arrays[k - d] : 0), ...);
        }
        __syncthreads();
#pragma unroll
        for (uint32_t r = 0; r < PER; r++) {
            const uint32_t k = t + NT * r;
            int i = 0;
            ((arrays[k] += x[r][i++]), ...);
        }
        __syncthreads();
    }
}

template <uint32_t NT, uint32_t BINS, class Bin, class Produce>
__device__ __forceinline__ void staged_counting_sort(uint32_t* stage, uint32_t* lstart, uint32_t* cur, uint32_t* goff, Bin bin, Produce produce,
                                                     uint32_t* __restrict__ out) {
    constexpr uint32_t PER = BINS / NT;
    static_assert(BINS == PER * NT && (BINS & (BINS - 1)) == 0, "staged_counting_sort: a power of two of bins, a whole number per lane");
    const uint32_t t = threadIdx.x;
    uint32_t mine[PER];
#pragma unroll
    for (uint32_t r = 0; r < PER; r++) {
        const uint2 b = bin(t + NT * r);
        mine[r] = b.x;
        goff[t + NT * r] = b.y;
        cur[t + NT * r] = b.x;
    }
    __syncthreads();
    block_scan_inclusive<NT, PER>(cur);
    uint32_t excl[PER];
#pragma unroll
    for (uint32_t r = 0; r < PER; r++) excl[r] = cur[t + NT * r] - mine[r];
    __syncthreads();
#pragma unroll
    for (uint32_t r = 0; r < PER; r++) lstart[t + NT * r] = excl[r];
#pragma unroll
    for (uint32_t r = 0; r < PER; r++) cur[t + NT * r] = excl[r];
    if (t == NT - 1) lstart[BINS] = excl[PER - 1] + mine[PER - 1];
    __syncthreads();
    const uint32_t total = produce([&](uint32_t k, uint32_t word) { stage[atomicAdd(&cur[k], 1u)] = word; });
    __syncthreads();
    for (uint32_t j = t; j < total; j += NT) {
        uint32_t k = 0;
#pragma unroll
        for (uint32_t step = BINS / 2; step >= 1; step >>= 1)
            if (lstart[k + step] <= j) k += step;
        out[goff[k] + (j - lstart[k])] = stage[j];
    }
}

struct WinGroup { uint32_t w0, w1, bin0, ncnt; };
__device__ __forceinline__ WinGroup window_group(const SortGeom& g, uint32_t grp) {
    const uint32_t wend = g.win0 + g.nwin;
    WinGroup r;
    r.w0 = g.win0 + grp * g.wgroup;
    r.w1 = r.w0 + g.wgroup < wend ? r.w0 + g.wgroup : wend;
    r.bin0 = g.shared ? 0u : (r.w0 - g.win0) * g.H;
    r.ncnt = (g.shared ? 1u : (r.w1 - r.w0)) * g.H;
    return r;
}

template <int CB, class Fn>
__device__ __forceinline__ void for_each_tile_digit(const uint32_t* __restrict__ scalars, const uint8_t* __restrict__ inf_flags, SortGeom g,
                                                    uint32_t tile, uint32_t nt, uint32_t w0, uint32_t w1, Fn f) {
    const uint32_t p0 = tile * g.tile_pts, p1 = p0 + g.tile_pts < g.n ? p0 + g.tile_pts : g.n;
    for (uint32_t i = p0 + threadIdx.x; i < p1; i += nt) {
        if (inf_flags[i] != 0) continue;
        uint32_t s[8];
        const bool flip = load_scalar(s, scalars, i, g.fmt);
        for_each_digit_static<CB>(s, flip, w0, w1, [&](uint32_t w, uint32_t b, bool neg) { f(i, w, b, neg); });
    }
}

__device__ __forceinline__ uint32_t coarse_entry(const SortGeom& g, uint32_t idx, uint32_t b, bool neg) {
    return (idx << (g.lo_bits + 1)) | ((neg ? 1u : 0u) << g.lo_bits) | (b & ((1u << g.lo_bits) - 1u));
}

template <bool SCATTER, int CB>
__global__ void __launch_bounds__(1024) k_coarse(const uint32_t* __restrict__ scalars, const uint8_t* __restrict__ inf_flags, SortGeom g,
                                                 uint32_t* __restrict__ tilecnt, const uint32_t* __restrict__ tileoff,
                                                 const uint32_t* __restrict__ bin_base, uint32_t* __restrict__ coarse) {
    aux_priority();
    __shared__ uint32_t cnt[SORT_MAX_COUNTERS];
    const uint32_t tile = blockIdx.x + g.tile0, t = threadIdx.x, nt = blockDim.x;
    const WinGroup wg = window_group(g, blockIdx.y);
    const size_t row = (size_t)tile * g.nbins + wg.bin0;
    for (uint32_t k = t; k < wg.ncnt; k += nt) cnt[k] = SCATTER ? bin_base[wg.bin0 + k] + tileoff[row + k] : 0u;
    __syncthreads();
    for_each_tile_digit<CB>(scalars, inf_flags, g, tile, nt, wg.w0, wg.w1, [&](uint32_t i, uint32_t w, uint32_t b, bool neg) {
        uint32_t k = (g.shared ? 0u : (w - wg.w0) * g.H) + (b >> g.lo_bits);
        uint32_t pos = atomicAdd(&cnt[k], 1u);
        if (SCATTER) coarse[pos] = coarse_entry(g, g.shared ? w * g.stride + i : i, b, neg);
    });
    if (!SCATTER) {
        __syncthreads();
        for (uint32_t k = t; k < wg.ncnt; k += nt) tilecnt[row + k] = cnt[k];
    }
}

constexpr uint32_t COARSE_STAGE = 16384;
constexpr uint32_t COARSE_STAGE_BINS = 512;
constexpr uint32_t COARSE_STAGE_CO = 14336;
constexpr uint32_t COARSE_STAGED_CO_LDS = (COARSE_STAGE_CO + 3 * COARSE_STAGE_BINS + 1) * 4;

template <int CB, uint32_t NT>
__device__ __forceinline__ void coarse_staged(uint32_t* stage, uint32_t* lstart, uint32_t* cur, uint32_t* goff, const uint32_t* __restrict__ scalars,
                                              const uint8_t* __restrict__ inf_flags, SortGeom g, const uint32_t* __restrict__ tilecnt,
                                              const uint32_t* __restrict__ tileoff, const uint32_t* __restrict__ bin_base, uint32_t* __restrict__ coarse) {
    const uint32_t tile = blockIdx.x;
    const WinGroup wg = window_group(g, blockIdx.y);
    const size_t row = (size_t)tile * g.nbins + wg.bin0;
    staged_counting_sort<NT, COARSE_STAGE_BINS>(
        stage, lstart, cur, goff,
        [&](uint32_t k) { return k < wg.ncnt ? make_uint2(tilecnt[row + k], bin_base[wg.bin0 + k] + tileoff[row + k]) : make_uint2(0u, 0u); },
        [&](auto emit) {
            const uint32_t total = lstart[COARSE_STAGE_BINS];
            for_each_tile_digit<CB>(scalars, inf_flags, g, tile, NT, wg.w0, wg.w1, [&](uint32_t i, uint32_t w, uint32_t b, bool neg) {
                emit((w - wg.w0) * g.H + (b >> g.lo_bits), coarse_entry(g, i, b, neg));
            });
            return total;
        },
        coarse);
}

template <int CB>
__global__ void __launch_bounds__(512) k_coarse_staged(const uint32_t* __restrict__ scalars, const uint8_t* __restrict__ inf_flags, SortGeom g,
                                                       const uint32_t* __restrict__ tilecnt, const uint32_t* __restrict__ tileoff,
                                                       const uint32_t* __restrict__ bin_base, uint32_t* __restrict__ coarse) {
    aux_priority();
    __shared__ uint32_t stage[COARSE_STAGE];
    __shared__ uint32_t lstart[COARSE_STAGE_BINS + 1], cur[COARSE_STAGE_BINS], goff[COARSE_STAGE_BINS];
    coarse_staged<CB, 512>(stage, lstart, cur, goff, scalars, inf_flags, g, tilecnt, tileoff, bin_base, coarse);
}

template <int CB>
__global__ void __launch_bounds__(256) k_coarse_staged_co(const uint32_t* __restrict__ scalars, const uint8_t* __restrict__ inf_flags, SortGeom g,
                                                          const uint32_t* __restrict__ tilecnt, const uint32_t* __restrict__ tileoff,
                                                          const uint32_t* __restrict__ bin_base, uint32_t* __restrict__ coarse) {
    aux_priority();
    extern __shared__ uint32_t dyn_lds[];
    uint32_t* const stage = dyn_lds;
    uint32_t* const lstart = stage + COARSE_STAGE_CO;
    uint32_t* const cur = lstart + COARSE_STAGE_BINS + 1;
    uint32_t* const goff = cur + COARSE_STAGE_BINS;
    coarse_staged<CB, 256>(stage, lstart, cur, goff, scalars, inf_flags, g, tilecnt, tileoff, bin_base, coarse);
}

__global__ void __launch_bounds__(256) k_colscan(const uint32_t* __restrict__ tilecnt, uint32_t nbins, uint32_t tiles,
                                                 uint32_t* __restrict__ tileoff, uint32_t* __restrict__ bin_tot) {
    aux_priority();
    uint32_t b = blockIdx.x * 256 + threadIdx.x;
    if (b >= nbins) return;
    uint32_t run = 0, k = 0;
    for (; k + 8 <= tiles; k += 8) {
        uint32_t v[8];
#pragma unroll
        for (int u = 0; u < 8; u++) v[u] = tilecnt[(size_t)(k + u) * nbins + b];
#pragma unroll
        for (int u = 0; u < 8; u++) {
            tileoff[(size_t)(k + u) * nbins + b] = run;
            run += v[u];
        }
    }
    for (; k < tiles; k++) {
        uint32_t v = tilecnt[(size_t)k * nbins + b];
        tileoff[(size_t)k * nbins + b] = run;
        run += v;
    }
    bin_tot[b] = run;
}

__global__ void __launch_bounds__(1024) k_binscan(const uint32_t* __restrict__ in, uint32_t m, uint32_t* __restrict__ out) {
    aux_priority();
    __shared__ uint32_t part[1024];
    uint32_t t = threadIdx.x;
    uint32_t per = (m + 1023) / 1024;
    uint32_t lo = t * per, hi = lo + per < m ? lo + per : m;
    uint32_t sum = 0;
    for (uint32_t k = lo; k < hi; k++) sum += in[k];
    part[t] = sum;
    __syncthreads();
    block_scan_inclusive<1024>(part);
    uint32_t run = part[t] - sum;
    for (uint32_t k = lo; k < hi; k++) {
        uint32_t v = in[k];
        out[k] = run;
        run += v;
    }
    if (t == 1023) out[m] = part[1023];
}

constexpr uint32_t FINE_SEG = 8192;
constexpr uint32_t FINE_SCATTER_LDS = (FINE_SEG + 257 + 256 + 256 + 4) * 4;

__global__ void __launch_bounds__(256) k_seg_count(const uint32_t* __restrict__ bin_base, uint32_t nbins, uint32_t* __restrict__ seg_cnt) {
    aux_priority();
    uint32_t b = blockIdx.x * 256 + threadIdx.x;
    if (b >= nbins) return;
    uint32_t sz = bin_base[b + 1] - bin_base[b];
    seg_cnt[b] = sz == 0 ? 1u : (sz + FINE_SEG - 1) / FINE_SEG;
}

__device__ __forceinline__ bool seg_locate(uint32_t seg, const uint32_t* seg_base, const uint32_t* bin_base, uint32_t nbins,
                                           uint32_t& bin, uint32_t& beg, uint32_t& end) {
    if (seg >= seg_base[nbins]) return false;
    uint32_t b = seg < nbins ? seg : nbins - 1;
    if (!(seg_base[b] <= seg && seg < seg_base[b + 1])) {
        uint32_t lo = 0, hi = b;
        while (lo < hi) {
            uint32_t mid = (lo + hi + 1) >> 1;
            if (seg_base[mid] <= seg) lo = mid; else hi = mid - 1;
        }
        b = lo;
    }
    uint32_t k = seg - seg_base[b];
    bin = b;
    beg = bin_base[b] + k * FINE_SEG;
    uint32_t bend = bin_base[b + 1];
    end = beg + FINE_SEG < bend ? beg + FINE_SEG : bend;
    return true;
}
struct Segment { uint32_t beg, end, bin_beg; };
template <bool BIN_BEG>
__device__ __forceinline__ bool seg_broadcast(uint32_t* sb, const uint32_t* seg_base, const uint32_t* bin_base, uint32_t nbins, Segment& s) {
    if (threadIdx.x == 0) {
        uint32_t bin = 0, beg = 0, end = 0;
        const bool ok = seg_locate(blockIdx.x, seg_base, bin_base, nbins, bin, beg, end);
        sb[0] = beg; sb[1] = end; sb[2] = ok ? 1u : 0u;
        if (BIN_BEG) sb[3] = ok ? bin_base[bin] : 0u;
    }
    __syncthreads();
    if (!sb[2]) return false;
    s.beg = sb[0]; s.end = sb[1]; s.bin_beg = BIN_BEG ? sb[3] : 0u;
    return true;
}

__global__ void __launch_bounds__(256) k_fine_count(const uint32_t* __restrict__ coarse, const uint32_t* __restrict__ bin_base,
                                                    const uint32_t* __restrict__ seg_base, SortGeom g, uint32_t* __restrict__ segcnt) {
    aux_priority();
    __shared__ uint32_t cnt[256];
    __shared__ uint32_t sb[3];
    uint32_t t = threadIdx.x, seg = blockIdx.x;
    cnt[t] = 0;
    Segment sg;
    if (!seg_broadcast<false>(sb, seg_base, bin_base, g.nbins, sg)) return;
    uint32_t beg = sg.beg, end = sg.end;
    uint32_t F = 1u << g.lo_bits, lo_mask = F - 1u;
    for (uint32_t i = beg + t; i < end; i += 256) atomicAdd(&cnt[coarse[i] & lo_mask], 1u);
    __syncthreads();
    if (t < F) segcnt[(size_t)seg * F + t] = cnt[t];
}

__global__ void __launch_bounds__(256) k_fine_scan(const uint32_t* __restrict__ seg_base, SortGeom g, const uint32_t* __restrict__ segcnt,
                                                   uint32_t* __restrict__ segoff, uint32_t* __restrict__ hist) {
    aux_priority();
    __shared__ uint32_t scan[256];
    uint32_t bin = blockIdx.x, t = threadIdx.x;
    uint32_t F = 1u << g.lo_bits;
    uint32_t s0 = seg_base[bin], s1 = seg_base[bin + 1];
    uint32_t tot = 0;
    if (t < F)
        for (uint32_t sg = s0; sg < s1; sg++) {
            uint32_t v = segcnt[(size_t)sg * F + t];
            segoff[(size_t)sg * F + t] = tot;
            tot += v;
        }
    scan[t] = t < F ? tot : 0;
    __syncthreads();
    block_scan_inclusive<256>(scan);
    if (t < F) {
        hist[(size_t)bin * F + t] = tot;
        uint32_t lo_base = scan[t] - tot;
        for (uint32_t sg = s0; sg < s1; sg++) segoff[(size_t)sg * F + t] += lo_base;
    }
}

__global__ void __launch_bounds__(256) k_fine_scatter(const uint32_t* __restrict__ coarse, const uint32_t* __restrict__ bin_base,
                                                      const uint32_t* __restrict__ seg_base, SortGeom g,
                                                      const uint32_t* __restrict__ segcnt, const uint32_t* __restrict__ segoff,
                                                      uint32_t* __restrict__ sorted) {
    aux_priority();
    extern __shared__ uint32_t dyn_lds[];
    uint32_t* const stage = dyn_lds;
    uint32_t* const lstart = stage + FINE_SEG;
    uint32_t* const cur = lstart + 257;
    uint32_t* const goff = cur + 256;
    uint32_t* const sb = goff + 256;
    const uint32_t t = threadIdx.x;
    Segment sg;
    if (!seg_broadcast<true>(sb, seg_base, bin_base, g.nbins, sg)) return;
    const uint32_t F = 1u << g.lo_bits, lo_mask = F - 1u, sh = g.lo_bits + 1;
    const size_t row = (size_t)blockIdx.x * F;
    staged_counting_sort<256, 256>(
        stage, lstart, cur, goff,
        [&](uint32_t k) { return k < F ? make_uint2(segcnt[row + k], sg.bin_beg + segoff[row + k]) : make_uint2(0u, 0u); },
        [&](auto emit) {
            for (uint32_t i = sg.beg + t; i < sg.end; i += 256) {
                const uint32_t e = coarse[i];
                emit(e & lo_mask, (e >> sh) | (((e >> g.lo_bits) & 1u) << 31));
            }
            return sg.end - sg.beg;
        },
        sorted);
}

constexpr uint32_t A_BITS = 5, A_BINS = 1u << A_BITS;
constexpr uint32_t MID_MAX = 512;
constexpr uint32_t MID_SCATTER_LDS = (8192 + 3 * MID_MAX + 1 + 4) * 4;

template <bool SCATTER, int CB>
__global__ void __launch_bounds__(1024) k_coarseA(const uint32_t* __restrict__ scalars, const uint8_t* __restrict__ inf_flags, SortGeom g,
                                                  uint32_t* __restrict__ tilecnt, const uint32_t* __restrict__ tileoff,
                                                  const uint32_t* __restrict__ binA_base, uint2* __restrict__ coarseA) {
    aux_priority();
    __shared__ uint32_t cnt[512];
    const uint32_t tile = blockIdx.x + g.tile0, t = threadIdx.x, nt = blockDim.x;
    const uint32_t nbinsA = g.nwin * A_BINS;
    for (uint32_t k = t; k < nbinsA; k += nt) cnt[k] = SCATTER ? binA_base[k] + tileoff[(size_t)tile * nbinsA + k] : 0u;
    __syncthreads();
    constexpr uint32_t REM = CB - 1 - A_BITS;
    for_each_tile_digit<CB>(scalars, inf_flags, g, tile, nt, g.win0, g.win0 + g.nwin, [&](uint32_t i, uint32_t w, uint32_t b, bool neg) {
        uint32_t pos = atomicAdd(&cnt[(w - g.win0) * A_BINS + (b >> REM)], 1u);
        if (SCATTER) coarseA[pos] = make_uint2(i, ((neg ? 1u : 0u) << 31) | (b & ((1u << REM) - 1u)));
    });
    if (!SCATTER) {
        __syncthreads();
        for (uint32_t k = t; k < nbinsA; k += nt) tilecnt[(size_t)tile * nbinsA + k] = cnt[k];
    }
}

__global__ void __launch_bounds__(256) k_mid_count(const uint2* __restrict__ coarseA, const uint32_t* __restrict__ binA_base,
                                                   const uint32_t* __restrict__ segA_base, uint32_t nbinsA, uint32_t lo_bits, uint32_t mid_bits,
                                                   uint32_t* __restrict__ segcnt) {
    aux_priority();
    __shared__ uint32_t cnt[MID_MAX];
    __shared__ uint32_t sb[3];
    uint32_t t = threadIdx.x, seg = blockIdx.x;
    cnt[t] = 0; cnt[t + 256] = 0;
    Segment sg;
    if (!seg_broadcast<false>(sb, segA_base, binA_base, nbinsA, sg)) return;
    const uint32_t beg = sg.beg, end = sg.end, M = 1u << mid_bits;
    for (uint32_t i = beg + t; i < end; i += 256) atomicAdd(&cnt[(coarseA[i].y >> lo_bits) & (M - 1u)], 1u);
    __syncthreads();
    for (uint32_t k = t; k < M; k += 256) segcnt[(size_t)seg * M + k] = cnt[k];
}

__global__ void __launch_bounds__(512) k_mid_scan(const uint32_t* __restrict__ binA_base, const uint32_t* __restrict__ segA_base,
                                                  uint32_t mid_bits, const uint32_t* __restrict__ segcnt, uint32_t* __restrict__ segoff,
                                                  uint32_t* __restrict__ bin_base, uint32_t nbinsA) {
    aux_priority();
    __shared__ uint32_t scan[MID_MAX];
    const uint32_t a = blockIdx.x, t = threadIdx.x, M = 1u << mid_bits;
    const uint32_t s0 = segA_base[a], s1 = segA_base[a + 1];
    uint32_t tot = 0;
    if (t < M) {
        uint32_t sg = s0;
        for (; sg + 8 <= s1; sg += 8) {
            uint32_t v[8];
#pragma unroll
            for (int u = 0; u < 8; u++) v[u] = segcnt[(size_t)(sg + u) * M + t];
#pragma unroll
            for (int u = 0; u < 8; u++) tot += v[u];
        }
        for (; sg < s1; sg++) tot += segcnt[(size_t)sg * M + t];
    }
    scan[t] = t < M ? tot : 0;
    __syncthreads();
    block_scan_inclusive<MID_MAX>(scan);
    if (t < M) {
        uint32_t run = scan[t] - tot;
        bin_base[(size_t)a * M + t] = binA_base[a] + run;
        uint32_t sg = s0;
        for (; sg + 8 <= s1; sg += 8) {
            uint32_t v[8];
#pragma unroll
            for (int u = 0; u < 8; u++) v[u] = segcnt[(size_t)(sg + u) * M + t];
#pragma unroll
            for (int u = 0; u < 8; u++) {
                segoff[(size_t)(sg + u) * M + t] = run;
                run += v[u];
            }
        }
        for (; sg < s1; sg++) {
            uint32_t v = segcnt[(size_t)sg * M + t];
            segoff[(size_t)sg * M + t] = run;
            run += v;
        }
    }
    if (a == nbinsA - 1 && t == 0) bin_base[(size_t)nbinsA * M] = binA_base[nbinsA];
}

__global__ void __launch_bounds__(256) k_mid_scatter(const uint2* __restrict__ coarseA, const uint32_t* __restrict__ binA_base,
                                                     const uint32_t* __restrict__ segA_base, uint32_t nbinsA, uint32_t lo_bits, uint32_t mid_bits,
                                                     const uint32_t* __restrict__ segcnt, const uint32_t* __restrict__ segoff,
                                                     uint32_t* __restrict__ coarse) {
    aux_priority();
    extern __shared__ uint32_t dyn_lds[];
    uint32_t* const stage = dyn_lds;
    uint32_t* const lstart = stage + FINE_SEG;
    uint32_t* const cur = lstart + MID_MAX + 1;
    uint32_t* const goff = cur + MID_MAX;
    uint32_t* const sb = goff + MID_MAX;
    const uint32_t t = threadIdx.x;
    Segment sg;
    if (!seg_broadcast<true>(sb, segA_base, binA_base, nbinsA, sg)) return;
    const uint32_t M = 1u << mid_bits, lo_mask = (1u << lo_bits) - 1u;
    const size_t row = (size_t)blockIdx.x * M;
    staged_counting_sort<256, MID_MAX>(
        stage, lstart, cur, goff,
        [&](uint32_t k) { return k < M ? make_uint2(segcnt[row + k], sg.bin_beg + segoff[row + k]) : make_uint2(0u, 0u); },
        [&](auto emit) {
            for (uint32_t i = sg.beg + t; i < sg.end; i += 256) {
                const uint2 e = coarseA[i];
                emit((e.y >> lo_bits) & (M - 1u), (e.x << (lo_bits + 1)) | ((e.y >> 31) << lo_bits) | (e.y & lo_mask));
            }
            return sg.end - sg.beg;
        },
        coarse);
}

constexpr int SCHED_CLASSES = 65;

__device__ __forceinline__ uint32_t items_of(uint32_t cnt, uint32_t logT, uint32_t logS) {
    const uint32_t lg = item_size_log(cnt, logT, logS);
    return cnt == 0 ? 1u : (cnt + (1u << lg) - 1u) >> lg;
}
__device__ __forceinline__ uint32_t last_len(uint32_t cnt, uint32_t it, uint32_t logS) { return it > 1 ? cnt - ((it - 1) << logS) : cnt; }
__device__ __forceinline__ uint32_t class_of(uint32_t len, uint32_t cls_shift) { uint32_t c = len >> cls_shift; return c < 64 ? c : 64; }

template <uint32_t NT>
__global__ void __launch_bounds__(NT) k_sched1(const uint32_t* __restrict__ hist, uint32_t m, uint32_t per_blk, uint32_t logT,
                                                 uint32_t nblk, uint32_t* __restrict__ blk_e, uint32_t* __restrict__ blk_i,
                                                 uint32_t* __restrict__ blk_cls, uint32_t* __restrict__ blk_max) {
    aux_priority();
    __shared__ uint32_t cls[SCHED_CLASSES];
    __shared__ uint32_t se, si, smax;
    uint32_t t = threadIdx.x, blk = blockIdx.x;
    if (t < SCHED_CLASSES) cls[t] = 0;
    if (t == 0) { se = 0; si = 0; smax = 1; }
    __syncthreads();
    uint32_t per_t = per_blk / NT;
    uint32_t lo = blk * per_blk + t * per_t, hi = lo + per_t < m ? lo + per_t : m;
    const uint32_t cls_shift = (logT >> 8) & 0xffu, logS = (logT >> 16) & 0xffu;
    logT &= 0xffu;
    uint32_t sum_e = 0, sum_i = 0, mx = 1;
    for (uint32_t k = lo; k < hi; k++) {
        uint32_t h = hist[k], it = items_of(h, logT, logS);
        sum_e += h;
        sum_i += it;
        mx = it > mx ? it : mx;
        if (it > 1) atomicAdd(&cls[64], it - 1);
        atomicAdd(&cls[class_of(last_len(h, it, logS), cls_shift)], 1u);
    }
    atomicAdd(&se, sum_e);
    atomicAdd(&si, sum_i);
    atomicMax(&smax, mx);
    __syncthreads();
    if (t < SCHED_CLASSES) blk_cls[t * nblk + blk] = cls[t];
    if (t == 0) { blk_e[blk] = se; blk_i[blk] = si; blk_max[blk] = smax; }
}

constexpr uint32_t SCHED_MAX_BLK = 1024;
template <uint32_t NT>
__global__ void __launch_bounds__(NT) k_sched2(uint32_t nblk, uint32_t* __restrict__ blk_e, uint32_t* __restrict__ blk_i,
                                                 uint32_t* __restrict__ blk_cls, const uint32_t* __restrict__ blk_max,
                                                 uint32_t* __restrict__ meta) {
    aux_priority();
    __shared__ uint32_t a[SCHED_MAX_BLK], b[SCHED_MAX_BLK], ctot[SCHED_CLASSES], cbase[SCHED_CLASSES];
    uint32_t t = threadIdx.x;
    constexpr uint32_t PER = SCHED_MAX_BLK / NT;
    static_assert(PER == 1 || PER == 2, "k_sched2: 512 or 1024 lanes");
    uint32_t ve[PER], vi[PER];
#pragma unroll
    for (uint32_t r = 0; r < PER; r++) {
        const uint32_t k = t + NT * r;
        ve[r] = k < nblk ? blk_e[k] : 0;
        vi[r] = k < nblk ? blk_i[k] : 0;
        a[k] = ve[r];
        b[k] = vi[r];
    }
    __syncthreads();
    block_scan_inclusive<NT, PER>(a, b);
#pragma unroll
    for (uint32_t r = 0; r < PER; r++) {
        const uint32_t k = t + NT * r;
        if (k < nblk) { blk_e[k] = a[k] - ve[r]; blk_i[k] = b[k] - vi[r]; }
    }
    uint32_t wave = t >> 6, lane = t & 63;
    for (uint32_t c = wave; c < SCHED_CLASSES; c += NT / 64) {
        uint32_t run = 0;
        for (uint32_t base = 0; base < nblk; base += 64) {
            uint32_t idx = base + lane;
            uint32_t v = idx < nblk ? blk_cls[c * nblk + idx] : 0, incl = v;
            for (int d = 1; d < 64; d <<= 1) {
                uint32_t u = __shfl_up(incl, d, 64);
                if ((int)lane >= d) incl += u;
            }
            if (idx < nblk) blk_cls[c * nblk + idx] = run + incl - v;
            run += __shfl(incl, 63, 64);
        }
        if (lane == 0) ctot[c] = run;
    }
    __syncthreads();
    if (t < SCHED_CLASSES) {
        uint32_t above = 0;
        for (uint32_t c = t + 1; c < SCHED_CLASSES; c++) above += ctot[c];
        cbase[t] = above;
    }
    __syncthreads();
    for (uint32_t idx = t; idx < SCHED_CLASSES * nblk; idx += NT) blk_cls[idx] += cbase[idx / nblk];
    if (t == 0) {
        uint32_t mx = 1;
        for (uint32_t k = 0; k < nblk; k++) mx = blk_max[k] > mx ? blk_max[k] : mx;
        meta[0] = b[SCHED_MAX_BLK - 1];
        meta[1] = mx;
        meta[2] = a[SCHED_MAX_BLK - 1];
        meta[3] = 0;
        meta[4] = 0;
        for (uint32_t k = 5; k < MERGE_META; k++) meta[k] = 0;
    }
}

template <uint32_t NT>
__global__ void __launch_bounds__(NT) k_sched3(const uint32_t* __restrict__ hist, uint32_t m, uint32_t per_blk, uint32_t logT,
                                                 uint32_t nblk, const uint32_t* __restrict__ blk_e, const uint32_t* __restrict__ blk_i,
                                                 const uint32_t* __restrict__ blk_cls, uint32_t* __restrict__ offsets,
                                                 uint32_t* __restrict__ woff,
                                                 uint32_t* __restrict__ order, uint32_t* __restrict__ item_bucket,
                                                 uint32_t* __restrict__ merge_list, uint32_t* __restrict__ meta) {
    aux_priority();
    __shared__ uint32_t pe[NT], pi[NT], cur[SCHED_CLASSES];
    constexpr uint32_t HV_CAP = 512, HV_MIN = 64;
    __shared__ uint32_t hv_k[HV_CAP], hv_run[HV_CAP], hv_it[HV_CAP], hv_pos[HV_CAP], hv_mp[HV_CAP], hv_n;
    uint32_t t = threadIdx.x, blk = blockIdx.x;
    if (t == 0) hv_n = 0;
    if (t < SCHED_CLASSES) cur[t] = blk_cls[t * nblk + blk];
    uint32_t per_t = per_blk / NT;
    uint32_t lo = blk * per_blk + t * per_t, hi = lo + per_t < m ? lo + per_t : m;
    const uint32_t cls_shift = (logT >> 8) & 0xffu, logS = (logT >> 16) & 0xffu;
    logT &= 0xffu;
    uint32_t sum_e = 0, sum_i = 0;
    for (uint32_t k = lo; k < hi; k++) {
        uint32_t h = hist[k];
        sum_e += h;
        sum_i += items_of(h, logT, logS);
    }
    pe[t] = sum_e;
    pi[t] = sum_i;
    __syncthreads();
    block_scan_inclusive<NT>(pe, pi);
    uint32_t run_e = blk_e[blk] + pe[t] - sum_e, run_i = blk_i[blk] + pi[t] - sum_i;
    for (uint32_t k = lo; k < hi; k++) {
        uint32_t h = hist[k], it = items_of(h, logT, logS);
        offsets[k] = run_e;
        woff[k] = run_i;
        if (it > 1) {
            uint32_t pos = atomicAdd(&cur[64], it - 1);
            uint32_t mp = atomicAdd(&meta[3], (it + MERGE_FAN - 1) / MERGE_FAN);
            atomicAdd(&meta[4], 1u);
            uint32_t slot = it >= HV_MIN ? atomicAdd(&hv_n, 1u) : HV_CAP;
            if (slot < HV_CAP) {
                hv_k[slot] = k; hv_run[slot] = run_i; hv_it[slot] = it; hv_pos[slot] = pos; hv_mp[slot] = mp;
            } else {
                for (uint32_t j = 0; j + 1 < it; j++) { order[pos + j] = run_i + j; item_bucket[run_i + j] = k; }
                for (uint32_t j = 0; j < it; j += MERGE_FAN) merge_list[mp + j / MERGE_FAN] = run_i + j;
            }
        }
        uint32_t last = run_i + it - 1;
        uint32_t pos = atomicAdd(&cur[class_of(last_len(h, it, logS), cls_shift)], 1u);
        order[pos] = last;
        item_bucket[last] = k;
        run_e += h;
        run_i += it;
    }
    if (blk == nblk - 1 && t == NT - 1) { offsets[m] = run_e; woff[m] = run_i; }
    __syncthreads();
    const uint32_t nh = hv_n < HV_CAP ? hv_n : HV_CAP;
    for (uint32_t s = 0; s < nh; s++) {
        const uint32_t k = hv_k[s], r0 = hv_run[s], it = hv_it[s], pos = hv_pos[s], mp = hv_mp[s];
        for (uint32_t j = t; j < it; j += NT) {
            if (j + 1 < it) { order[pos + j] = r0 + j; item_bucket[r0 + j] = k; }
            if (j % MERGE_FAN == 0) merge_list[mp + j / MERGE_FAN] = r0 + j;
        }
    }
}

}
```

Measured before the change: 343.2 million points/s.

## Fuse fine count and sort for single-segment bins and drop meta readback copy

Raises the fine segment size and fuses the fine count with a direct counting sort for bins that fit in one segment, so those bins skip the separate scan and scatter kernels. The segment-count and bin-base scans are merged into one kernel, and the fine kernels use a persistent grid-strided loop. The scheduler's last block writes meta counts straight to mapped host memory, replacing the separate D2H memcpy. This cuts kernel launches and global traffic in the sort phase, at the cost of extra LDS per block, more register pressure from holding segment entries, and a ticket-based last-block fence.

```diff
diff --git a/ark-blst_amd/binding.py b/ark-blst_amd/binding.py
--- a/ark-blst_amd/binding.py
+++ b/ark-blst_amd/binding.py
@@ -457,7 +457,7 @@
 
 
 def test_plan(n: int, forced_c: int = 0, group: str = "g1", shared: bool = False, stride: int = 0, fold: bool = False) -> dict:
-    out = (C.c_uint32 * 13)()
+    out = (C.c_uint32 * 14)()
     rc = load_library(True).mi_test_plan(n, forced_c, 0 if group == "g1" else 1, int(shared) | (2 if fold else 0), stride, out)
     if rc != 0:
         raise MsmError(rc, "mi_test_plan")
@@ -466,6 +466,7 @@
     d["nbuckets"] = (int(out[9]) << 32) | int(out[10])
     d["nchunks"] = int(out[11])
     d["serial_L"] = int(out[12])
+    d["fine_seg"] = int(out[13])
     d["serial_reduce"] = d["serial"]
     return d
 
diff --git a/ark-blst_amd/csrc/api.hip b/ark-blst_amd/csrc/api.hip
--- a/ark-blst_amd/csrc/api.hip
+++ b/ark-blst_amd/csrc/api.hip
@@ -467,7 +467,7 @@
     Plan p = make_plan(n, forced_c, group == 0 ? g1_cost() : g2_cost(), (shared & 1) != 0, stride, (shared & 2) != 0);
     out[0] = p.c; out[1] = p.nwin; out[2] = p.bwin; out[3] = p.coop_L; out[4] = p.chunk_buckets; out[5] = p.logT; out[6] = p.lo_bits;
     out[7] = p.serial_reduce ? 1u : 0u; out[8] = p.chunks_per_win; out[9] = (uint32_t)(p.nbuckets >> 32); out[10] = (uint32_t)p.nbuckets;
-    out[11] = (uint32_t)p.nchunks; out[12] = p.serial_reduce ? p.serial_L : 0u;
+    out[11] = (uint32_t)p.nchunks; out[12] = p.serial_reduce ? p.serial_L : 0u; out[13] = p.fine_seg;
     return MI_OK;
 }
 #endif
diff --git a/ark-blst_amd/csrc/common.hpp b/ark-blst_amd/csrc/common.hpp
--- a/ark-blst_amd/csrc/common.hpp
+++ b/ark-blst_amd/csrc/common.hpp
@@ -57,6 +57,7 @@
     uint32_t chunk_buckets;
     bool serial_reduce;
     uint32_t serial_L;
+    uint32_t fine_seg;
 };
 
 struct DevBuf {
@@ -140,6 +141,7 @@
     DevBuf hist, offsets, woff, meta, sched, sorted, partial, order, item_bucket, pairs, pairs2;
     DevBuf tilecnt, tileoff, bin_tot, bin_base, binA_base, coarse, coarseA, seg_cnt, seg_base, segcnt, segoff, merge_list, merge_list2;
     uint32_t* h_meta = nullptr;
+    uint32_t* h_meta_dev = nullptr;
     hipEvent_t ev[8] = {};
     template <class Fn> void for_each_buf(Fn fn) {
         for (DevBuf* b : {&hist, &offsets, &woff, &meta, &sched, &sorted, &partial, &order, &item_bucket, &pairs, &pairs2, &tilecnt, &tileoff, &bin_tot,
diff --git a/ark-blst_amd/csrc/kernels_common.cuh b/ark-blst_amd/csrc/kernels_common.cuh
--- a/ark-blst_amd/csrc/kernels_common.cuh
+++ b/ark-blst_amd/csrc/kernels_common.cuh
@@ -194,6 +194,7 @@
 
 constexpr uint32_t MERGE_FAN = 4;
 constexpr uint32_t MERGE_META = 32;
+constexpr uint32_t SCHED_TICKET = 5;
 constexpr uint32_t CLK_META = 24;
 
 struct WaveClock {
diff --git a/ark-blst_amd/csrc/msm_sort.hip b/ark-blst_amd/csrc/msm_sort.hip
--- a/ark-blst_amd/csrc/msm_sort.hip
+++ b/ark-blst_amd/csrc/msm_sort.hip
@@ -71,6 +71,7 @@
         uint32_t lo_bits = std::min<uint32_t>(std::min<uint32_t>(8, c - 1), 31 - idx_bits);
         if (((1u << (c - 1)) >> lo_bits) > msmk::SORT_MAX_COUNTERS) continue;
         p.lo_bits = lo_bits;
+        p.fine_seg = msmk::FINE_SEG;
         if ((uint64_t)n * p.nwin >= (1ull << 32)) continue;
         p.nb = 1u << (c - 1);
         p.bwin = shared ? 1 : p.nwin;
@@ -214,7 +215,10 @@
     sc.woff.ensure((pl.nbuckets + 1) * 4);
     sc.meta.ensure(msmk::MERGE_META * 4);
     sc.sorted.ensure(entries_cap * 4);
-    if (!sc.h_meta) HIP_TRY(hipHostMalloc((void**)&sc.h_meta, 32, hipHostMallocDefault));
+    if (!sc.h_meta) {
+        HIP_TRY(hipHostMalloc((void**)&sc.h_meta, 32, hipHostMallocDefault));
+        HIP_TRY(hipHostGetDevicePointer((void**)&sc.h_meta_dev, sc.h_meta, 0));
+    }
 
     const bool phases = d.prof_level >= 2;
     if (phases) HIP_TRY(hipEventRecord(sc.ev[0], s));
@@ -254,7 +258,7 @@
         size_t seg_words = (size_t)segs_cap * (1u << g.lo_bits), bins = g.nbins;
         if (three_level) {
             const uint32_t nbinsA = pl.nwin * msmk::A_BINS;
-            const size_t segs_capA = nbinsA + entries_cap / msmk::FINE_SEG + 1;
+            const size_t segs_capA = nbinsA + entries_cap / msmk::MID_SEG + 1;
             seg_words = std::max(seg_words, segs_capA << ((pl.c - 1 - msmk::A_BITS) - pl.lo_bits));
             bins = std::max<size_t>(bins, nbinsA);
         }
@@ -263,6 +267,10 @@
         sc.segcnt.ensure(seg_words * 4);
         sc.segoff.ensure(seg_words * 4);
     }
+    auto segment_bases = [&](const uint32_t* bases, uint32_t bins, uint32_t seg) {
+        hipLaunchKernelGGL(msmk::k_seg_count, dim3((bins + 255) / 256), dim3(256), 0, s, bases, bins, seg, (uint32_t*)sc.seg_cnt.p);
+        hipLaunchKernelGGL(msmk::k_binscan, dim3(1), dim3(1024), 0, s, (const uint32_t*)sc.seg_cnt.p, bins, (uint32_t*)sc.seg_base.p);
+    };
     if (three_level) {
         const uint32_t nbinsA = pl.nwin * msmk::A_BINS;
         const uint32_t mid_bits = (pl.c - 1 - msmk::A_BITS) - pl.lo_bits, M = 1u << mid_bits;
@@ -270,7 +278,7 @@
         g.wgroup = pl.nwin; g.ngroups = 1;
         g.tile_pts = (uint32_t)std::min<size_t>(8192, (n + 1023) / 1024 * 1024);
         g.tiles = (uint32_t)((n + g.tile_pts - 1) / g.tile_pts);
-        const uint32_t segs_capA = nbinsA + (uint32_t)(entries_cap / msmk::FINE_SEG) + 1;
+        const uint32_t segs_capA = nbinsA + (uint32_t)(entries_cap / msmk::MID_SEG) + 1;
         sc.tilecnt.ensure((size_t)g.tiles * nbinsA * 4);
         sc.tileoff.ensure((size_t)g.tiles * nbinsA * 4);
         sc.bin_tot.ensure((size_t)nbinsA * 4);
@@ -285,9 +293,7 @@
         hipLaunchKernelGGL(msmk::k_binscan, dim3(1), dim3(1024), 0, s, (const uint32_t*)sc.bin_tot.p, nbinsA, (uint32_t*)sc.binA_base.p);
         launch_coarseA<true>(pl.c, dim3(g.tiles), digit_block_big, s, d_scalars, d_flags, g, (uint32_t*)sc.tilecnt.p, (const uint32_t*)sc.tileoff.p,
                              (const uint32_t*)sc.binA_base.p, (uint2*)sc.coarseA.p);
-        hipLaunchKernelGGL(msmk::k_seg_count, dim3((nbinsA + 255) / 256), dim3(256), 0, s, (const uint32_t*)sc.binA_base.p, nbinsA,
-                           (uint32_t*)sc.seg_cnt.p);
-        hipLaunchKernelGGL(msmk::k_binscan, dim3(1), dim3(1024), 0, s, (const uint32_t*)sc.seg_cnt.p, nbinsA, (uint32_t*)sc.seg_base.p);
+        segment_bases((const uint32_t*)sc.binA_base.p, nbinsA, msmk::MID_SEG);
         hipLaunchKernelGGL(msmk::k_mid_count, dim3(segs_capA), dim3(256), 0, s, (const uint2*)sc.coarseA.p, (const uint32_t*)sc.binA_base.p,
                            (const uint32_t*)sc.seg_base.p, nbinsA, pl.lo_bits, mid_bits, (uint32_t*)sc.segcnt.p);
         hipLaunchKernelGGL(msmk::k_mid_scan, dim3(nbinsA), dim3(512), 0, s, (const uint32_t*)sc.binA_base.p, (const uint32_t*)sc.seg_base.p, mid_bits,
@@ -295,6 +301,7 @@
         hipLaunchKernelGGL(msmk::k_mid_scatter, dim3(segs_capA), dim3(256), msmk::MID_SCATTER_LDS, s, (const uint2*)sc.coarseA.p, (const uint32_t*)sc.binA_base.p,
                            (const uint32_t*)sc.seg_base.p, nbinsA, pl.lo_bits, mid_bits, (const uint32_t*)sc.segcnt.p, (const uint32_t*)sc.segoff.p,
                            (uint32_t*)sc.coarse.p);
+        segment_bases((const uint32_t*)sc.bin_base.p, g.nbins, msmk::FINE_SEG);
     } else {
     const bool staged = !shared_buckets && g.H <= 128 && pl.c <= 16 && n >= 4096;
     uint32_t coarse_block;
@@ -319,7 +326,8 @@
     });
     hipLaunchKernelGGL(msmk::k_colscan, dim3((g.nbins + 255) / 256), dim3(256), 0, s, (const uint32_t*)sc.tilecnt.p, g.nbins, g.tiles,
                        (uint32_t*)sc.tileoff.p, (uint32_t*)sc.bin_tot.p);
-    hipLaunchKernelGGL(msmk::k_binscan, dim3(1), dim3(1024), 0, s, (const uint32_t*)sc.bin_tot.p, g.nbins, (uint32_t*)sc.bin_base.p);
+    hipLaunchKernelGGL(msmk::k_bin_seg_scan, dim3(1), dim3(msmk::BINSEG_NT), 0, s, (const uint32_t*)sc.bin_tot.p, g.nbins, (uint32_t*)sc.bin_base.p,
+                       msmk::FINE_SEG, (uint32_t*)sc.seg_base.p);
     if (staged)
         launch_coarse_staged(pl.c, under_accumulate, dim3(g.tiles, g.ngroups), s, d_scalars, d_flags, g, (const uint32_t*)sc.tilecnt.p, (const uint32_t*)sc.tileoff.p,
                              (const uint32_t*)sc.bin_base.p, (uint32_t*)sc.coarse.p);
@@ -328,14 +336,12 @@
                             (const uint32_t*)sc.tileoff.p, (const uint32_t*)sc.bin_base.p, (uint32_t*)sc.coarse.p);
     }
     if (phases) HIP_TRY(hipEventRecord(sc.ev[1], s));
-    hipLaunchKernelGGL(msmk::k_seg_count, dim3((g.nbins + 255) / 256), dim3(256), 0, s, (const uint32_t*)sc.bin_base.p, g.nbins,
-                       (uint32_t*)sc.seg_cnt.p);
-    hipLaunchKernelGGL(msmk::k_binscan, dim3(1), dim3(1024), 0, s, (const uint32_t*)sc.seg_cnt.p, g.nbins, (uint32_t*)sc.seg_base.p);
-    hipLaunchKernelGGL(msmk::k_fine_count, dim3(segs_cap), dim3(256), 0, s, (const uint32_t*)sc.coarse.p, (const uint32_t*)sc.bin_base.p,
-                       (const uint32_t*)sc.seg_base.p, g, (uint32_t*)sc.segcnt.p);
+    const uint32_t fine_grid = std::min(segs_cap, msmk::FINE_GRID);
+    hipLaunchKernelGGL(msmk::k_fine_count_sort, dim3(fine_grid), dim3(256), msmk::FINE_SEG_LDS, s, (const uint32_t*)sc.coarse.p, (const uint32_t*)sc.bin_base.p,
+                       (const uint32_t*)sc.seg_base.p, g, (uint32_t*)sc.segcnt.p, (uint32_t*)sc.hist.p, (uint32_t*)sc.sorted.p);
     hipLaunchKernelGGL(msmk::k_fine_scan, dim3(g.nbins), dim3(256), 0, s, (const uint32_t*)sc.seg_base.p, g, (const uint32_t*)sc.segcnt.p,
                        (uint32_t*)sc.segoff.p, (uint32_t*)sc.hist.p);
-    hipLaunchKernelGGL(msmk::k_fine_scatter, dim3(segs_cap), dim3(256), msmk::FINE_SCATTER_LDS, s, (const uint32_t*)sc.coarse.p, (const uint32_t*)sc.bin_base.p,
+    hipLaunchKernelGGL(msmk::k_fine_scatter, dim3(fine_grid), dim3(256), msmk::FINE_SCATTER_LDS, s, (const uint32_t*)sc.coarse.p, (const uint32_t*)sc.bin_base.p,
                        (const uint32_t*)sc.seg_base.p, g, (const uint32_t*)sc.segcnt.p, (const uint32_t*)sc.segoff.p, (uint32_t*)sc.sorted.p);
     if (phases) HIP_TRY(hipEventRecord(sc.ev[2], s));
     const uint32_t sched_nt = under_accumulate ? 512 : 1024;
@@ -361,11 +367,10 @@
         hipLaunchKernelGGL(msmk::k_sched2<NT>, dim3(1), dim3(NT), 0, s, nblk, blk_e, blk_i, blk_cls, (const uint32_t*)blk_max, (uint32_t*)sc.meta.p);
         hipLaunchKernelGGL(msmk::k_sched3<NT>, dim3(nblk), dim3(NT), 0, s, (const uint32_t*)sc.hist.p, (uint32_t)pl.nbuckets, per_blk, packed, nblk, (const uint32_t*)blk_e,
                            (const uint32_t*)blk_i, (const uint32_t*)blk_cls, (uint32_t*)sc.offsets.p, (uint32_t*)sc.woff.p, (uint32_t*)sc.order.p,
-                           (uint32_t*)sc.item_bucket.p, (uint32_t*)sc.merge_list.p, (uint32_t*)sc.meta.p);
+                           (uint32_t*)sc.item_bucket.p, (uint32_t*)sc.merge_list.p, (uint32_t*)sc.meta.p, sc.h_meta_dev);
     };
     if (under_accumulate) schedule(std::integral_constant<uint32_t, 512>{});
     else schedule(std::integral_constant<uint32_t, 1024>{});
-    HIP_TRY(hipMemcpyAsync(sc.h_meta, sc.meta.p, 32, hipMemcpyDeviceToHost, s));
     HIP_TRY(hipEventRecord(sc.ev[3], s));
 }
 
diff --git a/ark-blst_amd/csrc/sort_kernels.cuh b/ark-blst_amd/csrc/sort_kernels.cuh
--- a/ark-blst_amd/csrc/sort_kernels.cuh
+++ b/ark-blst_amd/csrc/sort_kernels.cuh
@@ -37,7 +37,7 @@
     }
 }
 
-template <uint32_t NT, uint32_t BINS, class Bin, class Produce>
+template <uint32_t NT, uint32_t BINS, bool REL = false, class Bin, class Produce>
 __device__ __forceinline__ void staged_counting_sort(uint32_t* stage, uint32_t* lstart, uint32_t* cur, uint32_t* goff, Bin bin, Produce produce,
                                                      uint32_t* __restrict__ out) {
     constexpr uint32_t PER = BINS / NT;
@@ -56,6 +56,10 @@
     uint32_t excl[PER];
 #pragma unroll
     for (uint32_t r = 0; r < PER; r++) excl[r] = cur[t + NT * r] - mine[r];
+    if (REL) {
+#pragma unroll
+        for (uint32_t r = 0; r < PER; r++) goff[t + NT * r] += excl[r];
+    }
     __syncthreads();
 #pragma unroll
     for (uint32_t r = 0; r < PER; r++) lstart[t + NT * r] = excl[r];
@@ -171,6 +175,29 @@
     coarse_staged<CB, 256>(stage, lstart, cur, goff, scalars, inf_flags, g, tilecnt, tileoff, bin_base, coarse);
 }
 
+__device__ __forceinline__ bool last_block_out(uint32_t* ticket, uint32_t* flag) {
+    asm volatile("s_waitcnt vmcnt(0)" ::: "memory");
+    __syncthreads();
+    if (threadIdx.x == 0) {
+        __builtin_amdgcn_fence(__ATOMIC_RELEASE, "agent");
+        asm volatile("s_waitcnt vmcnt(0)" ::: "memory");
+        const bool last = __hip_atomic_fetch_add(ticket, 1u, __ATOMIC_RELAXED, __HIP_MEMORY_SCOPE_AGENT) == gridDim.x * gridDim.y - 1u;
+        if (last) {
+            __hip_atomic_store(ticket, 0u, __ATOMIC_RELAXED, __HIP_MEMORY_SCOPE_AGENT);
+            __builtin_amdgcn_fence(__ATOMIC_ACQUIRE, "agent");
+            asm volatile("s_waitcnt vmcnt(0)" ::: "memory");
+        }
+        *flag = last ? 1u : 0u;
+    }
+    __syncthreads();
+    return *flag != 0;
+}
+__device__ __forceinline__ uint32_t load_agent(const uint32_t* p) {
+    return __hip_atomic_load(const_cast<uint32_t*>(p), __ATOMIC_RELAXED, __HIP_MEMORY_SCOPE_AGENT);
+}
+
+__device__ __forceinline__ uint32_t segments_of(uint32_t sz, uint32_t seg) { return sz == 0 ? 1u : (sz + seg - 1) / seg; }
+
 __global__ void __launch_bounds__(256) k_colscan(const uint32_t* __restrict__ tilecnt, uint32_t nbins, uint32_t tiles,
                                                  uint32_t* __restrict__ tileoff, uint32_t* __restrict__ bin_tot) {
     aux_priority();
@@ -215,18 +242,54 @@
     if (t == 1023) out[m] = part[1023];
 }
 
-constexpr uint32_t FINE_SEG = 8192;
-constexpr uint32_t FINE_SCATTER_LDS = (FINE_SEG + 257 + 256 + 256 + 4) * 4;
-
-__global__ void __launch_bounds__(256) k_seg_count(const uint32_t* __restrict__ bin_base, uint32_t nbins, uint32_t* __restrict__ seg_cnt) {
+constexpr uint32_t BINSEG_NT = 512;
+__global__ void __launch_bounds__(BINSEG_NT) k_bin_seg_scan(const uint32_t* __restrict__ bin_tot, uint32_t m, uint32_t* __restrict__ bin_base,
+                                                            uint32_t seg, uint32_t* __restrict__ seg_base) {
+    aux_priority();
+    __shared__ uint32_t part[BINSEG_NT], part2[BINSEG_NT];
+    const uint32_t t = threadIdx.x;
+    const uint32_t per = (m + BINSEG_NT - 1) / BINSEG_NT;
+    const uint32_t lo = t * per < m ? t * per : m, hi = lo + per < m ? lo + per : m;
+    uint32_t sum = 0, ssum = 0;
+    for (uint32_t k = lo; k < hi; k++) {
+        const uint32_t v = bin_tot[k];
+        sum += v;
+        ssum += segments_of(v, seg);
+    }
+    part[t] = sum;
+    part2[t] = ssum;
+    __syncthreads();
+    block_scan_inclusive<BINSEG_NT>(part, part2);
+    uint32_t run = part[t] - sum, srun = part2[t] - ssum;
+    for (uint32_t k = lo; k < hi; k++) {
+        const uint32_t v = bin_tot[k];
+        bin_base[k] = run;
+        seg_base[k] = srun;
+        run += v;
+        srun += segments_of(v, seg);
+    }
+    if (t == BINSEG_NT - 1) {
+        bin_base[m] = part[BINSEG_NT - 1];
+        seg_base[m] = part2[BINSEG_NT - 1];
+    }
+}
+
+constexpr uint32_t FINE_SEG = 8960;
+constexpr uint32_t FINE_PER = FINE_SEG / 256;
+static_assert(FINE_SEG % 256 == 0, "FINE_SEG: a whole number of entries per lane");
+constexpr uint32_t FINE_SCATTER_LDS = (FINE_SEG + 257 + 256 + 256 + 8) * 4;
+constexpr uint32_t FINE_SEG_LDS = FINE_SCATTER_LDS + 256 * 4;
+static_assert(FINE_SEG_LDS <= 65536, "k_fine_count_sort: dynamic LDS beyond what a plain launch may ask for");
+constexpr uint32_t FINE_GRID = 2048;
+
+__global__ void __launch_bounds__(256) k_seg_count(const uint32_t* __restrict__ bin_base, uint32_t nbins, uint32_t seg, uint32_t* __restrict__ seg_cnt) {
     aux_priority();
     uint32_t b = blockIdx.x * 256 + threadIdx.x;
     if (b >= nbins) return;
-    uint32_t sz = bin_base[b + 1] - bin_base[b];
-    seg_cnt[b] = sz == 0 ? 1u : (sz + FINE_SEG - 1) / FINE_SEG;
-}
-
-__device__ __forceinline__ bool seg_locate(uint32_t seg, const uint32_t* seg_base, const uint32_t* bin_base, uint32_t nbins,
+    seg_cnt[b] = segments_of(bin_base[b + 1] - bin_base[b], seg);
+}
+
+__device__ __forceinline__ bool seg_locate(uint32_t seg, const uint32_t* seg_base, const uint32_t* bin_base, uint32_t nbins, uint32_t SEG,
                                            uint32_t& bin, uint32_t& beg, uint32_t& end) {
     if (seg >= seg_base[nbins]) return false;
     uint32_t b = seg < nbins ? seg : nbins - 1;
@@ -240,40 +303,78 @@
     }
     uint32_t k = seg - seg_base[b];
     bin = b;
-    beg = bin_base[b] + k * FINE_SEG;
+    beg = bin_base[b] + k * SEG;
     uint32_t bend = bin_base[b + 1];
-    end = beg + FINE_SEG < bend ? beg + FINE_SEG : bend;
+    end = beg + SEG < bend ? beg + SEG : bend;
     return true;
 }
-struct Segment { uint32_t beg, end, bin_beg; };
-template <bool BIN_BEG>
-__device__ __forceinline__ bool seg_broadcast(uint32_t* sb, const uint32_t* seg_base, const uint32_t* bin_base, uint32_t nbins, Segment& s) {
+struct Segment {
+    uint32_t beg, end;
+    uint32_t bin, bin_beg;
+    bool single;
+};
+__device__ __forceinline__ bool seg_broadcast(uint32_t* sb, uint32_t seg, const uint32_t* seg_base, const uint32_t* bin_base, uint32_t nbins, uint32_t SEG,
+                                              Segment& s) {
     if (threadIdx.x == 0) {
         uint32_t bin = 0, beg = 0, end = 0;
-        const bool ok = seg_locate(blockIdx.x, seg_base, bin_base, nbins, bin, beg, end);
-        sb[0] = beg; sb[1] = end; sb[2] = ok ? 1u : 0u;
-        if (BIN_BEG) sb[3] = ok ? bin_base[bin] : 0u;
+        const bool ok = seg_locate(seg, seg_base, bin_base, nbins, SEG, bin, beg, end);
+        sb[0] = beg; sb[1] = end; sb[2] = ok ? 1u : 0u; sb[3] = bin;
+        sb[4] = ok ? bin_base[bin] : 0u;
+        sb[5] = ok && seg_base[bin + 1] - seg_base[bin] == 1u ? 1u : 0u;
     }
     __syncthreads();
     if (!sb[2]) return false;
-    s.beg = sb[0]; s.end = sb[1]; s.bin_beg = BIN_BEG ? sb[3] : 0u;
+    s.beg = sb[0]; s.end = sb[1]; s.bin = sb[3]; s.bin_beg = sb[4]; s.single = sb[5] != 0;
     return true;
 }
 
-__global__ void __launch_bounds__(256) k_fine_count(const uint32_t* __restrict__ coarse, const uint32_t* __restrict__ bin_base,
-                                                    const uint32_t* __restrict__ seg_base, SortGeom g, uint32_t* __restrict__ segcnt) {
-    aux_priority();
-    __shared__ uint32_t cnt[256];
-    __shared__ uint32_t sb[3];
-    uint32_t t = threadIdx.x, seg = blockIdx.x;
-    cnt[t] = 0;
-    Segment sg;
-    if (!seg_broadcast<false>(sb, seg_base, bin_base, g.nbins, sg)) return;
-    uint32_t beg = sg.beg, end = sg.end;
-    uint32_t F = 1u << g.lo_bits, lo_mask = F - 1u;
-    for (uint32_t i = beg + t; i < end; i += 256) atomicAdd(&cnt[coarse[i] & lo_mask], 1u);
-    __syncthreads();
-    if (t < F) segcnt[(size_t)seg * F + t] = cnt[t];
+__device__ __forceinline__ uint32_t sorted_entry(const SortGeom& g, uint32_t e) { return (e >> (g.lo_bits + 1)) | (((e >> g.lo_bits) & 1u) << 31); }
+
+__global__ void __launch_bounds__(256) k_fine_count_sort(const uint32_t* __restrict__ coarse, const uint32_t* __restrict__ bin_base,
+                                                  const uint32_t* __restrict__ seg_base, SortGeom g, uint32_t* __restrict__ segcnt,
+                                                  uint32_t* __restrict__ hist, uint32_t* __restrict__ sorted) {
+    aux_priority();
+    extern __shared__ uint32_t dyn_lds[];
+    uint32_t* const stage = dyn_lds;
+    uint32_t* const lstart = stage + FINE_SEG;
+    uint32_t* const cur = lstart + 257;
+    uint32_t* const goff = cur + 256;
+    uint32_t* const sb = goff + 256;
+    uint32_t* const cnt = sb + 8;
+    const uint32_t t = threadIdx.x;
+    const uint32_t F = 1u << g.lo_bits, lo_mask = F - 1u;
+    const uint32_t nsegs = seg_base[g.nbins];
+    for (uint32_t seg = blockIdx.x; seg < nsegs; seg += gridDim.x) {
+        cnt[t] = 0;
+        Segment sg;
+        if (!seg_broadcast(sb, seg, seg_base, bin_base, g.nbins, FINE_SEG, sg)) return;
+        const uint32_t len = sg.end - sg.beg;
+        uint32_t mine = len > t ? (len - t + 255) / 256 : 0u;
+        uint32_t e[FINE_PER];
+#pragma unroll
+        for (uint32_t r = 0; r < FINE_PER; r++) e[r] = r < mine ? coarse[sg.beg + t + 256 * r] : 0u;
+        asm volatile("" : "+v"(mine));
+#pragma unroll
+        for (uint32_t r = 0; r < FINE_PER; r++)
+            if (r < mine) atomicAdd(&cnt[e[r] & lo_mask], 1u);
+        asm volatile("" : "+v"(mine));
+        __syncthreads();
+        if (!sg.single) {
+            if (t < F) segcnt[(size_t)seg * F + t] = cnt[t];
+            continue;
+        }
+        if (t < F) hist[(size_t)sg.bin * F + t] = cnt[t];
+        staged_counting_sort<256, 256, true>(
+            stage, lstart, cur, goff,
+            [&](uint32_t k) { return k < F ? make_uint2(cnt[k], sg.bin_beg) : make_uint2(0u, 0u); },
+            [&](auto emit) {
+#pragma unroll
+                for (uint32_t r = 0; r < FINE_PER; r++)
+                    if (r < mine) emit(e[r] & lo_mask, sorted_entry(g, e[r]));
+                return len;
+            },
+            sorted);
+    }
 }
 
 __global__ void __launch_bounds__(256) k_fine_scan(const uint32_t* __restrict__ seg_base, SortGeom g, const uint32_t* __restrict__ segcnt,
@@ -282,7 +383,9 @@
     __shared__ uint32_t scan[256];
     uint32_t bin = blockIdx.x, t = threadIdx.x;
     uint32_t F = 1u << g.lo_bits;
+    if (seg_base[g.nbins] == g.nbins) return;
     uint32_t s0 = seg_base[bin], s1 = seg_base[bin + 1];
+    if (s1 - s0 == 1) return;
     uint32_t tot = 0;
     if (t < F)
         for (uint32_t sg = s0; sg < s1; sg++) {
@@ -312,26 +415,39 @@
     uint32_t* const goff = cur + 256;
     uint32_t* const sb = goff + 256;
     const uint32_t t = threadIdx.x;
-    Segment sg;
-    if (!seg_broadcast<true>(sb, seg_base, bin_base, g.nbins, sg)) return;
-    const uint32_t F = 1u << g.lo_bits, lo_mask = F - 1u, sh = g.lo_bits + 1;
-    const size_t row = (size_t)blockIdx.x * F;
-    staged_counting_sort<256, 256>(
-        stage, lstart, cur, goff,
-        [&](uint32_t k) { return k < F ? make_uint2(segcnt[row + k], sg.bin_beg + segoff[row + k]) : make_uint2(0u, 0u); },
-        [&](auto emit) {
-            for (uint32_t i = sg.beg + t; i < sg.end; i += 256) {
-                const uint32_t e = coarse[i];
-                emit(e & lo_mask, (e >> sh) | (((e >> g.lo_bits) & 1u) << 31));
-            }
-            return sg.end - sg.beg;
-        },
-        sorted);
+    const uint32_t F = 1u << g.lo_bits, lo_mask = F - 1u;
+    const uint32_t nsegs = seg_base[g.nbins];
+    if (nsegs == g.nbins) return;
+    for (uint32_t seg = blockIdx.x; seg < nsegs; seg += gridDim.x) {
+        {
+            const uint32_t b = seg < g.nbins ? seg : g.nbins - 1;
+            if (seg_base[b] == seg && seg_base[b + 1] == seg + 1) continue;
+        }
+        Segment sg;
+        if (!seg_broadcast(sb, seg, seg_base, bin_base, g.nbins, FINE_SEG, sg)) return;
+        if (sg.single) {
+            __syncthreads();
+            continue;
+        }
+        const size_t row = (size_t)seg * F;
+        staged_counting_sort<256, 256>(
+            stage, lstart, cur, goff,
+            [&](uint32_t k) { return k < F ? make_uint2(segcnt[row + k], sg.bin_beg + segoff[row + k]) : make_uint2(0u, 0u); },
+            [&](auto emit) {
+                for (uint32_t i = sg.beg + t; i < sg.end; i += 256) {
+                    const uint32_t e = coarse[i];
+                    emit(e & lo_mask, sorted_entry(g, e));
+                }
+                return sg.end - sg.beg;
+            },
+            sorted);
+    }
 }
 
 constexpr uint32_t A_BITS = 5, A_BINS = 1u << A_BITS;
 constexpr uint32_t MID_MAX = 512;
-constexpr uint32_t MID_SCATTER_LDS = (8192 + 3 * MID_MAX + 1 + 4) * 4;
+constexpr uint32_t MID_SEG = 8192;
+constexpr uint32_t MID_SCATTER_LDS = (MID_SEG + 3 * MID_MAX + 1 + 8) * 4;
 
 template <bool SCATTER, int CB>
 __global__ void __launch_bounds__(1024) k_coarseA(const uint32_t* __restrict__ scalars, const uint8_t* __restrict__ inf_flags, SortGeom g,
@@ -359,11 +475,11 @@
                                                    uint32_t* __restrict__ segcnt) {
     aux_priority();
     __shared__ uint32_t cnt[MID_MAX];
-    __shared__ uint32_t sb[3];
+    __shared__ uint32_t sb[8];
     uint32_t t = threadIdx.x, seg = blockIdx.x;
     cnt[t] = 0; cnt[t + 256] = 0;
     Segment sg;
-    if (!seg_broadcast<false>(sb, segA_base, binA_base, nbinsA, sg)) return;
+    if (!seg_broadcast(sb, blockIdx.x, segA_base, binA_base, nbinsA, MID_SEG, sg)) return;
     const uint32_t beg = sg.beg, end = sg.end, M = 1u << mid_bits;
     for (uint32_t i = beg + t; i < end; i += 256) atomicAdd(&cnt[(coarseA[i].y >> lo_bits) & (M - 1u)], 1u);
     __syncthreads();
@@ -422,13 +538,13 @@
     aux_priority();
     extern __shared__ uint32_t dyn_lds[];
     uint32_t* const stage = dyn_lds;
-    uint32_t* const lstart = stage + FINE_SEG;
+    uint32_t* const lstart = stage + MID_SEG;
     uint32_t* const cur = lstart + MID_MAX + 1;
     uint32_t* const goff = cur + MID_MAX;
     uint32_t* const sb = goff + MID_MAX;
     const uint32_t t = threadIdx.x;
     Segment sg;
-    if (!seg_broadcast<true>(sb, segA_base, binA_base, nbinsA, sg)) return;
+    if (!seg_broadcast(sb, blockIdx.x, segA_base, binA_base, nbinsA, MID_SEG, sg)) return;
     const uint32_t M = 1u << mid_bits, lo_mask = (1u << lo_bits) - 1u;
     const size_t row = (size_t)blockIdx.x * M;
     staged_counting_sort<256, MID_MAX>(
@@ -552,9 +668,9 @@
                                                  const uint32_t* __restrict__ blk_cls, uint32_t* __restrict__ offsets,
                                                  uint32_t* __restrict__ woff,
                                                  uint32_t* __restrict__ order, uint32_t* __restrict__ item_bucket,
-                                                 uint32_t* __restrict__ merge_list, uint32_t* __restrict__ meta) {
-    aux_priority();
-    __shared__ uint32_t pe[NT], pi[NT], cur[SCHED_CLASSES];
+                                                 uint32_t* __restrict__ merge_list, uint32_t* meta, uint32_t* host_counts) {
+    aux_priority();
+    __shared__ uint32_t pe[NT], pi[NT], cur[SCHED_CLASSES], last;
     constexpr uint32_t HV_CAP = 512, HV_MIN = 64;
     __shared__ uint32_t hv_k[HV_CAP], hv_run[HV_CAP], hv_it[HV_CAP], hv_pos[HV_CAP], hv_mp[HV_CAP], hv_n;
     uint32_t t = threadIdx.x, blk = blockIdx.x;
@@ -608,6 +724,7 @@
             if (j % MERGE_FAN == 0) merge_list[mp + j / MERGE_FAN] = r0 + j;
         }
     }
-}
-
-}
+    if (last_block_out(meta + SCHED_TICKET, &last) && t < 5) host_counts[t] = load_agent(meta + t);
+}
+
+}
```

After: 346.0 million points/s (median of 6 runs). About the same (+0.8%).
